# EnyaHermite/SPH3D-GCN

Hardware: AMD Instinct MI355X
Metric: point-cloud blocks/sec (fwd+bwd) SPH3D_s3dis 8192-pt (higher is better)
Workload: dtype f32

## Files before the change

### include/sph3d.h

```cpp
#ifndef SPH3D_H
#define SPH3D_H

#include <stddef.h>

#ifdef __cplusplus
extern "C" {
#endif

typedef void* sph3d_stream_t;

enum {
    SPH3D_OK = 0,
    SPH3D_EINVAL = -1,
    SPH3D_EWORKSPACE = -2,
    SPH3D_ELAUNCH = -3,
    SPH3D_EUNSUPPORTED = -4
};

#define SPH3D_ABI_VERSION 2
int sph3d_abi_version(void);
const char* sph3d_last_error(void);
const char* sph3d_build_info(void);


#define SPH3D_MAX_GROWTH_PASSES 4096
long long sph3d_nngrid_launches(void);
int sph3d_build_sphere_neighbor(int B, int N, int M, int nn_sample, float radius,
                                const float* database, const float* query,
                                int* nn_index, int* nn_count, float* nn_dist,
                                sph3d_stream_t stream);
int sph3d_build_sphere_neighbor_fixed(int B, int N, int M, int nn_sample, float radius,
                                const float* database, const float* query,
                                int* nn_index, int* nn_count, float* nn_dist,
                                sph3d_stream_t stream);

size_t sph3d_build_sphere_neighbor_workspace(int B, int N, int M);
int sph3d_build_sphere_neighbor_ws(int B, int N, int M, int nn_sample, float radius,
                                   const float* database, const float* query,
                                   int* nn_index, int* nn_count, float* nn_dist,
                                   void* workspace, size_t workspace_bytes, sph3d_stream_t stream);
int sph3d_build_sphere_neighbor_fixed_ws(int B, int N, int M, int nn_sample, float radius,
                                   const float* database, const float* query,
                                   int* nn_index, int* nn_count, float* nn_dist,
                                   void* workspace, size_t workspace_bytes, sph3d_stream_t stream);
int sph3d_release_stream_scratch(sph3d_stream_t stream);
int sph3d_release_all_scratch(void);

int sph3d_build_cube_neighbor(int B, int N, int M, int grid_size, int nn_sample, float length,
                              const float* database, const float* query,
                              int* nn_index, int* nn_count,
                              sph3d_stream_t stream);

int sph3d_build_sphere_graph(int B, int N, int M, int nn_sample, float radius, int n, int p, int q,
                             const float* database, const float* query,
                             int* nn_index, int* nn_count, float* nn_dist, int* filt_index,
                             void* transpose_workspace, size_t transpose_workspace_bytes, sph3d_stream_t stream);
int sph3d_build_sphere_graph_ocml(int B, int N, int M, int nn_sample, float radius, int n, int p, int q,
                             const float* database, const float* query,
                             int* nn_index, int* nn_count, float* nn_dist, int* filt_index,
                             void* transpose_workspace, size_t transpose_workspace_bytes, sph3d_stream_t stream);

int sph3d_build_sphere_graph_ws(int B, int N, int M, int nn_sample, float radius, int n, int p, int q, int ocml,
                                const float* database, const float* query,
                                int* nn_index, int* nn_count, float* nn_dist, int* filt_index,
                                void* transpose_workspace, size_t transpose_workspace_bytes,
                                void* search_workspace, size_t search_workspace_bytes, sph3d_stream_t stream);

int sph3d_spherical_kernel(int B, int N, int M, int K, int n, int p, int q, float radius,
                           const float* database, const float* query,
                           const int* nn_index, const int* nn_count, const float* nn_dist,
                           int* filt_index,
                           sph3d_stream_t stream);
int sph3d_spherical_kernel_ocml(int B, int N, int M, int K, int n, int p, int q, float radius,
                                const float* database, const float* query,
                                const int* nn_index, const int* nn_count, const float* nn_dist,
                                int* filt_index,
                                sph3d_stream_t stream);

int sph3d_depthwise_conv3d(int B, int N, int M, int F, int C, int r, int K,
                           const int* nn_index, const int* nn_count, const int* bin_index,
                           const float* input, const float* filter, float* output,
                           sph3d_stream_t stream);

size_t sph3d_depthwise_conv3d_grad_workspace(int B, int N, int M, int F, int C, int r, int K);
int sph3d_depthwise_conv3d_grad(int B, int N, int M, int F, int C, int r, int K,
                                const int* nn_index, const int* nn_count, const int* bin_index,
                                const float* input, const float* filter, const float* grad_output,
                                float* grad_input, float* grad_filter,
                                void* workspace, size_t workspace_bytes,
                                sph3d_stream_t stream);

size_t sph3d_graph_transpose_workspace(int B, int N, int M, int K, int F);
int sph3d_graph_transpose(int B, int N, int M, int K, int F,
                          const int* nn_index, const int* nn_count,
                          const int* bin_index , const float* weight ,
                          int* offsets, int* ent_key, float* ent_scale,
                          int* active_bins ,
                          void* workspace, size_t workspace_bytes, sph3d_stream_t stream);
int sph3d_graph_transpose_count(int B, int N, int M, int K, int F, const int* nn_index, const int* nn_count,
                                const int* bin_index, int want_active, void* workspace, size_t workspace_bytes,
                                sph3d_stream_t stream);
int sph3d_graph_transpose_finish(int B, int N, int M, int K, int F,
                                 const int* nn_index, const int* nn_count, const int* bin_index,
                                 const float* weight, int* offsets, int* ent_key, float* ent_scale, int* active_bins,
                                 void* workspace, size_t workspace_bytes, sph3d_stream_t stream);
int sph3d_gather_rows_count(int B, int N, int S, int K, const int* pairs, const int* nn_index, const int* nn_count,
                            int* out_index, int* out_count, void* transpose_workspace, size_t transpose_workspace_bytes,
                            sph3d_stream_t stream);
int sph3d_graph_transpose_finish_ordered(int B, int N, int M, int K, int F,
                                         const int* nn_index, const int* nn_count, const int* bin_index,
                                         const float* weight, int* offsets, int* ent_key, float* ent_scale, int* active_bins,
                                         int* order, void* workspace, size_t workspace_bytes, sph3d_stream_t stream);
int sph3d_graph_balanced_order(int B, int N, int F, const int* offsets, int* order, sph3d_stream_t stream);
size_t sph3d_depthwise_conv3d_grad_t_workspace(int B, int N, int F, int C, int r);
int sph3d_depthwise_conv3d_grad_t(int B, int N, int M, int F, int C, int r,
                                  const int* offsets, const int* ent_key, const float* ent_scale,
                                  const int* source_order ,
                                  const int* active_bins ,
                                  const float* input, const float* filter, const float* grad_output,
                                  float* grad_input, float* grad_filter,
                                  void* workspace, size_t workspace_bytes, sph3d_stream_t stream);
int sph3d_scatter_grad_t(int B, int Nin, int Mout, int C,
                         const int* offsets, const int* ent_key, const float* ent_scale,
                         const float* grad_output, float* grad_input, sph3d_stream_t stream);
size_t sph3d_scatter_grad_workspace(int B, int N, int M, int K);

int sph3d_max_pool3d(int B, int N, int M, int C, int K,
                     const int* nn_index, const int* nn_count, const float* input,
                     float* output, int* max_index, sph3d_stream_t stream);
int sph3d_max_pool3d_grad(int B, int N, int M, int C,
                          const int* max_index, const float* grad_output,
                          float* grad_input, sph3d_stream_t stream);
int sph3d_max_pool3d_grad_t(int B, int N, int M, int C, const int* offsets, const int* ent_key, const int* nn_count,
                            const int* max_index, const float* grad_output,
                            const float* addend ,
                            float* grad_input, sph3d_stream_t stream);
int sph3d_avg_pool3d(int B, int N, int M, int C, int K,
                     const int* nn_index, const int* nn_count, const float* input,
                     float* output, sph3d_stream_t stream);
int sph3d_avg_pool3d_grad(int B, int N, int M, int C, int K,
                          const int* nn_index, const int* nn_count, const float* grad_output,
                          float* grad_input,
                          void* workspace , size_t workspace_bytes,
                          sph3d_stream_t stream);

int sph3d_mean_interpolate(int B, int N, int M, int C, int K,
                           const int* nn_index, const int* nn_count, const float* input,
                           float* output, sph3d_stream_t stream);
int sph3d_mean_interpolate_grad(int B, int N, int M, int C, int K,
                                const int* nn_index, const int* nn_count, const float* grad_output,
                                float* grad_input,
                                void* workspace , size_t workspace_bytes,
                                sph3d_stream_t stream);
int sph3d_weighted_interpolate(int B, int N, int M, int C, int K,
                               const int* nn_index, const int* nn_count,
                               const float* input, const float* weight,
                               float* output, sph3d_stream_t stream);
int sph3d_weighted_interpolate_grad(int B, int N, int M, int C, int K,
                                    const int* nn_index, const int* nn_count,
                                    const float* grad_output, const float* weight,
                                    float* grad_input,
                                    void* workspace , size_t workspace_bytes,
                                    sph3d_stream_t stream);

size_t sph3d_farthest_point_sample_workspace(int b, int n, int m);
int sph3d_farthest_point_sample(int b, int n, int m, const float* inp, int* out,
                                void* workspace, size_t workspace_bytes,
                                sph3d_stream_t stream);

int sph3d_gather_nd(int B, int N, long long S, int row, const int* pairs, const void* params, void* out,
                    sph3d_stream_t stream);

int sph3d_spatial_order(int B, int N, const float* xyz, int* order, sph3d_stream_t stream);

int sph3d_pointwise_gemm(int R, int Cin, int Cout,
                         const float* X, const float* W, const float* bias, int act,
                         int trans_w, float* Y, sph3d_stream_t stream);
int sph3d_pointwise_gemm_mode(int mode);
int sph3d_pointwise_gemm_exchange_failures(void);
int sph3d_pointwise_gemm_tn(int R, int Cin, int Cout,
                            const float* X, const float* dY, float* dW,
                            void* workspace, size_t workspace_bytes,
                            sph3d_stream_t stream);
size_t sph3d_pointwise_gemm_tn_workspace(int R, int Cin, int Cout);

size_t sph3d_elu_bn_workspace(int R, int C);
int sph3d_elu_bn_forward(int R, int C, const float* y, const float* gamma, const float* beta,
                         float* running_mean, float* running_var, float momentum, float eps, int training,
                         float* out, float* save_mean, float* save_rstd,
                         void* workspace, size_t workspace_bytes, sph3d_stream_t stream);
int sph3d_elu_bn_backward(int R, int C, const float* y, const float* dout, const float* gamma,
                          const float* save_mean, const float* save_rstd, int training,
                          float* dy, float* dgamma, float* dbeta,
                          void* workspace, size_t workspace_bytes, sph3d_stream_t stream);

int sph3d_pointwise_gemm_bnstats_blocks(int R, int Cin, int Cout);
int sph3d_pointwise_gemm_bnstats(int R, int Cin, int Cout, const float* X, const float* W, const float* bias ,
                                 float* Y, float* partial, sph3d_stream_t stream);
int sph3d_elu_bn_forward_partials(int R, int C, int nblk, const float* partial, const float* y, const float* gamma,
                                  const float* beta, float* running_mean, float* running_var, float momentum, float eps,
                                  float* out, float* save_mean, float* save_rstd, sph3d_stream_t stream);

int sph3d_separable_conv3d_fused_supported(int N, int F, int C, int r, int K, int Cout);
int sph3d_separable_conv3d_fused(int B, int N, int M, int F, int C, int r, int K, int Cout, int act,
                                 const int* nn_index, const int* nn_count, const int* bin_index, const float* input,
                                 const float* depthwise_filter, const float* pointwise_weights, const float* bias,
                                 const float* scale, const float* shift, float* output, sph3d_stream_t stream);

int sph3d_separable_conv3d_train_supported(int N, int F, int C, int r, int K, int Cout);
int sph3d_separable_conv3d_train_blocks(int Cout);
int sph3d_separable_conv3d_train(int B, int N, int M, int F, int C, int r, int K, int Cout,
                                 const int* nn_index, const int* nn_count, const int* bin_index, const float* input,
                                 const float* depthwise_filter, const float* pointwise_weights, const float* bias,
                                 float* depthwise_output, float* y, float* partial, sph3d_stream_t stream);
int sph3d_separable_conv3d_ring_failures(void);

int sph3d_pointwise_gemm_skinny_supported(int R, int K1, int K2, int N);
int sph3d_pointwise_gemm_skinny(int R, int K1, int K2, int N, const float* A1, const float* A2, const float* W, const float* bias,
                                float* Y, sph3d_stream_t stream);
size_t sph3d_pointwise_gemm_skinny_tn_workspace(int R, int K1, int K2, int N);
int sph3d_pointwise_gemm_skinny_tn(int R, int K1, int K2, int N, const float* A1, const float* A2, const float* dY, float* dW,
                                   void* workspace, size_t workspace_bytes, sph3d_stream_t stream);

int sph3d_depthwise_conv3d_cat_supported(int F, int Ca, int Cb, int r);
int sph3d_depthwise_conv3d_cat(int B, int N, int M, int F, int Ca, int Cb, int r, int K, const int* nn_index, const int* nn_count,
                               const int* bin_index, const float* input_a, const float* input_b, const float* filter, float* output,
                               sph3d_stream_t stream);
int sph3d_depthwise_conv3d_grad_t_cat(int B, int N, int M, int F, int Ca, int Cb, int r, const int* offsets, const int* ent_key,
                                      const float* ent_scale, const int* source_order, const int* active_bins, const float* input_a,
                                      const float* input_b, const float* filter, const float* grad_output, float* grad_a,
                                      float* grad_b, float* grad_filter, void* workspace, size_t workspace_bytes,
                                      sph3d_stream_t stream);

int sph3d_adam_step(long long n, float* param, const float* grad, float* exp_avg, float* exp_avg_sq, float lr, float beta1,
                    float beta2, float eps, int step, sph3d_stream_t stream);

int sph3d_feed_assemble(int B, int num_point, int num_blocks, long long total_rows, const float* rows, const long long* offsets,
                        const int* block_ids, unsigned long long seed, unsigned long long step, int augment, float* points,
                        int* label, int* inner, int* index, sph3d_stream_t stream);

size_t sph3d_vote_workspace(long long batch_rows);
int sph3d_vote_begin(int B, int C, int num_blocks, long long total_rows, const float* rows, const long long* offsets,
                     const int* block_ids, long long row_base, long long batch_rows, float* votes, int* count, int* covered,
                     int* inner_size, int* remaining, void* workspace, size_t workspace_bytes, sph3d_stream_t stream);
int sph3d_vote_accumulate(int B, int num_point, int C, int num_blocks, long long total_rows, const float* rows,
                          const long long* offsets, const int* block_ids, long long row_base, long long batch_rows, int pass,
                          const int* index, const float* logits, int min_votes, float* votes, int* count, int* covered,
                          const int* inner_size, int* remaining, void* workspace, size_t workspace_bytes, sph3d_stream_t stream);
int sph3d_vote_finalize(int B, int C, int num_blocks, long long total_rows, const float* rows, const long long* offsets,
                        const int* block_ids, long long row_base, long long batch_rows, const float* votes, int* pred,
                        long long* confusion, long long* nonfinite, sph3d_stream_t stream);

#define SPH3D_NN1_GRID 0
#define SPH3D_NN1_BRUTE 1
int sph3d_scene_merge(int B, int C, int num_blocks, long long total_rows, const float* rows, const long long* offsets,
                      const int* index, const int* block_ids, long long row_base, long long batch_rows, const float* votes,
                      long long V, float* merged, int* hits, long long* counters, sph3d_stream_t stream);
int sph3d_scene_finalize(int C, long long V, const float* merged, const int* hits, const int* voxel_label, int* pred_voxel,
                         long long* unseen_rows, long long* confusion, sph3d_stream_t stream);
size_t sph3d_nn1_workspace(long long V, long long F);
int sph3d_nn1(long long V, long long F, const float* ref_xyz, const float* query_xyz, int mode, int* idx, void* workspace,
              size_t workspace_bytes, sph3d_stream_t stream);
int sph3d_scene_lift(int C, long long V, long long F, const int* pred_voxel, const int* idx, const int* label_map,
                     const int* label_full, int* pred_full, long long* confusion, sph3d_stream_t stream);

#define SPH3D_PREP_REDUCE_ATOMIC 0
#define SPH3D_PREP_REDUCE_SORTED 1
size_t sph3d_prep_voxel_grid_workspace(long long F, long long max_cells);
int sph3d_prep_voxel_grid(long long F, int A, const float* xyz, const float* attr, float h, long long max_cells,
                          int* voxel_of_point, int* header, void* workspace, size_t workspace_bytes, sph3d_stream_t stream);
size_t sph3d_prep_voxel_reduce_workspace(long long F, long long V, int mode);
int sph3d_prep_voxel_reduce(long long F, int A, long long V, const float* xyz, const float* attr, const int* voxel_of_point,
                            int mode, long long* sums, int* count, void* workspace, size_t workspace_bytes, sph3d_stream_t stream);
int sph3d_prep_voxel_finalize(long long V, int A, const long long* sums, const int* count, float* voxel_xyz, float* voxel_attr,
                              int* box, sph3d_stream_t stream);
int sph3d_prep_box(long long V, const float* xyz, int* box, sph3d_stream_t stream);
int sph3d_prep_normalise(long long V, const float* voxel_xyz, const float* voxel_rgb, const int* box, float* out_xyz,
                         float* out_rgb, sph3d_stream_t stream);
int sph3d_prep_rect_count(long long V, int R, const float* xyz, const float* rects, int* counts, sph3d_stream_t stream);
size_t sph3d_prep_block_fill_workspace(long long V, int P);
int sph3d_prep_block_fill(long long V, int P, long long T, const float* xyz, const float* rgb, const int* label,
                          const float* rects, const long long* offsets, float* rows, int* index, int* mismatch, void* workspace,
                          size_t workspace_bytes, sph3d_stream_t stream);

int sph3d_masked_softmax_xent_parts(int N);
int sph3d_masked_softmax_xent(int B, int N, int C, const float* logits, const long long* label, const float* inner_label,
                              float* loss_part, float* dlogits, sph3d_stream_t stream);

#ifdef __cplusplus
}
#endif
#endif
```

### sph3d_gcn_amd/_lib.py

```python
import ctypes
import os

import torch

_HERE = os.path.dirname(os.path.abspath(__file__))
LIB_PATH = os.environ.get("SPH3D_LIB") or os.path.join(_HERE, "csrc", "libsph3d.so")

_c_int = ctypes.c_int
_c_float = ctypes.c_float
_c_size_t = ctypes.c_size_t
_vp = ctypes.c_void_p

_I, _F, _P, _S, _L = _c_int, _c_float, _vp, _c_size_t, ctypes.c_longlong
SIGNATURES = {
    "sph3d_abi_version": (_I, []),
    "sph3d_last_error": (ctypes.c_char_p, []),
    "sph3d_build_info": (ctypes.c_char_p, []),
    "sph3d_build_sphere_neighbor": (_I, [_I, _I, _I, _I, _F, _P, _P, _P, _P, _P, _P]),
    "sph3d_build_sphere_neighbor_fixed": (_I, [_I, _I, _I, _I, _F, _P, _P, _P, _P, _P, _P]),
    "sph3d_build_sphere_neighbor_workspace": (_S, [_I, _I, _I]),
    "sph3d_build_sphere_neighbor_ws": (_I, [_I, _I, _I, _I, _F, _P, _P, _P, _P, _P, _P, _S, _P]),
    "sph3d_build_sphere_neighbor_fixed_ws": (_I, [_I, _I, _I, _I, _F, _P, _P, _P, _P, _P, _P, _S, _P]),
    "sph3d_release_stream_scratch": (_I, [_P]),
    "sph3d_release_all_scratch": (_I, []),
    "sph3d_build_sphere_graph_ws": (_I, [_I, _I, _I, _I, _F, _I, _I, _I, _I] + [_P] * 6 + [_P, _S, _P, _S, _P]),
    "sph3d_build_cube_neighbor": (_I, [_I, _I, _I, _I, _I, _F, _P, _P, _P, _P, _P]),
    "sph3d_spherical_kernel": (_I, [_I, _I, _I, _I, _I, _I, _I, _F, _P, _P, _P, _P, _P, _P, _P]),
    "sph3d_spherical_kernel_ocml": (_I, [_I, _I, _I, _I, _I, _I, _I, _F, _P, _P, _P, _P, _P, _P, _P]),
    "sph3d_depthwise_conv3d": (_I, [_I] * 7 + [_P] * 7),
    "sph3d_depthwise_conv3d_grad_workspace": (_S, [_I] * 7),
    "sph3d_depthwise_conv3d_grad": (_I, [_I] * 7 + [_P] * 8 + [_P, _S, _P]),
    "sph3d_max_pool3d": (_I, [_I] * 5 + [_P] * 6),
    "sph3d_max_pool3d_grad": (_I, [_I] * 4 + [_P] * 4),
    "sph3d_max_pool3d_grad_t": (_I, [_I] * 4 + [_P] * 8),
    "sph3d_avg_pool3d": (_I, [_I] * 5 + [_P] * 5),
    "sph3d_avg_pool3d_grad": (_I, [_I] * 5 + [_P] * 4 + [_P, _S, _P]),
    "sph3d_graph_balanced_order": (_I, [_I, _I, _I, _P, _P, _P]),
    "sph3d_gather_nd": (_I, [_I, _I, ctypes.c_longlong, _I, _P, _P, _P, _P]),
    "sph3d_gather_rows_count": (_I, [_I] * 4 + [_P] * 5 + [_P, _S, _P]),
    "sph3d_graph_transpose_workspace": (_S, [_I] * 5),
    "sph3d_graph_transpose": (_I, [_I] * 5 + [_P] * 8 + [_P, _S, _P]),
    "sph3d_graph_transpose_count": (_I, [_I] * 5 + [_P] * 3 + [_I, _P, _S, _P]),
    "sph3d_graph_transpose_finish": (_I, [_I] * 5 + [_P] * 8 + [_P, _S, _P]),
    "sph3d_graph_transpose_finish_ordered": (_I, [_I] * 5 + [_P] * 9 + [_P, _S, _P]),
    "sph3d_build_sphere_graph": (_I, [_I, _I, _I, _I, _F, _I, _I, _I] + [_P] * 6 + [_P, _S, _P]),
    "sph3d_build_sphere_graph_ocml": (_I, [_I, _I, _I, _I, _F, _I, _I, _I] + [_P] * 6 + [_P, _S, _P]),
    "sph3d_depthwise_conv3d_grad_t_workspace": (_S, [_I] * 5),
    "sph3d_depthwise_conv3d_grad_t": (_I, [_I] * 6 + [_P] * 10 + [_P, _S, _P]),
    "sph3d_depthwise_conv3d_cat_supported": (_I, [_I] * 4),
    "sph3d_depthwise_conv3d_cat": (_I, [_I] * 8 + [_P] * 8),
    "sph3d_depthwise_conv3d_grad_t_cat": (_I, [_I] * 7 + [_P] * 12 + [_P, _S, _P]),
    "sph3d_spatial_order": (_I, [_I, _I, _P, _P, _P]),
    "sph3d_scatter_grad_t": (_I, [_I] * 4 + [_P] * 6),
    "sph3d_scatter_grad_workspace": (_S, [_I] * 4),
    "sph3d_mean_interpolate": (_I, [_I] * 5 + [_P] * 5),
    "sph3d_mean_interpolate_grad": (_I, [_I] * 5 + [_P] * 4 + [_P, _S, _P]),
    "sph3d_weighted_interpolate": (_I, [_I] * 5 + [_P] * 6),
    "sph3d_weighted_interpolate_grad": (_I, [_I] * 5 + [_P] * 5 + [_P, _S, _P]),
    "sph3d_farthest_point_sample_workspace": (_S, [_I] * 3),
    "sph3d_farthest_point_sample": (_I, [_I] * 3 + [_P, _P, _P, _S, _P]),
    "sph3d_pointwise_gemm": (_I, [_I] * 3 + [_P, _P, _P, _I, _I, _P, _P]),
    "sph3d_pointwise_gemm_mode": (_I, [_I]),
    "sph3d_pointwise_gemm_tn_workspace": (_S, [_I] * 3),
    "sph3d_pointwise_gemm_tn": (_I, [_I] * 3 + [_P, _P, _P, _P, _S, _P]),
    "sph3d_elu_bn_workspace": (_S, [_I] * 2),
    "sph3d_pointwise_gemm_bnstats_blocks": (_I, [_I] * 3),
    "sph3d_pointwise_gemm_bnstats": (_I, [_I] * 3 + [_P] * 6),
    "sph3d_nngrid_launches": (ctypes.c_longlong, []),
    "sph3d_masked_softmax_xent_parts": (_I, [_I]),
    "sph3d_masked_softmax_xent": (_I, [_I, _I, _I] + [_P] * 5 + [_P]),
    "sph3d_adam_step": (_I, [ctypes.c_longlong] + [_P] * 4 + [_F] * 4 + [_I, _P]),
    "sph3d_feed_assemble": (_I, [_I, _I, _I, ctypes.c_longlong, _P, _P, _P, ctypes.c_ulonglong, ctypes.c_ulonglong, _I] + [_P] * 5),
    "sph3d_vote_workspace": (_S, [ctypes.c_longlong]),
    "sph3d_vote_begin": (_I, [_I, _I, _I, ctypes.c_longlong, _P, _P, _P, ctypes.c_longlong, ctypes.c_longlong] + [_P] * 5 + [_P, _S, _P]),
    "sph3d_vote_accumulate": (_I, [_I, _I, _I, _I, ctypes.c_longlong, _P, _P, _P, ctypes.c_longlong, ctypes.c_longlong, _I, _P, _P, _I]
                              + [_P] * 5 + [_P, _S, _P]),
    "sph3d_vote_finalize": (_I, [_I, _I, _I, ctypes.c_longlong, _P, _P, _P, ctypes.c_longlong, ctypes.c_longlong] + [_P] * 4 + [_P]),
    "sph3d_scene_merge": (_I, [_I, _I, _I, _L, _P, _P, _P, _P, _L, _L, _P, _L, _P, _P, _P, _P]),
    "sph3d_scene_finalize": (_I, [_I, _L] + [_P] * 6 + [_P]),
    "sph3d_nn1_workspace": (_S, [_L, _L]),
    "sph3d_nn1": (_I, [_L, _L, _P, _P, _I, _P, _P, _S, _P]),
    "sph3d_scene_lift": (_I, [_I, _L, _L] + [_P] * 6 + [_P]),
    "sph3d_prep_voxel_grid_workspace": (_S, [_L, _L]),
    "sph3d_prep_voxel_grid": (_I, [_L, _I, _P, _P, _F, _L, _P, _P, _P, _S, _P]),
    "sph3d_prep_voxel_reduce_workspace": (_S, [_L, _L, _I]),
    "sph3d_prep_voxel_reduce": (_I, [_L, _I, _L, _P, _P, _P, _I, _P, _P, _P, _S, _P]),
    "sph3d_prep_voxel_finalize": (_I, [_L, _I] + [_P] * 5 + [_P]),
    "sph3d_prep_box": (_I, [_L, _P, _P, _P]),
    "sph3d_prep_normalise": (_I, [_L] + [_P] * 5 + [_P]),
    "sph3d_prep_rect_count": (_I, [_L, _I, _P, _P, _P, _P]),
    "sph3d_prep_block_fill_workspace": (_S, [_L, _I]),
    "sph3d_prep_block_fill": (_I, [_L, _I, _L] + [_P] * 8 + [_P, _S, _P]),
    "sph3d_pointwise_gemm_skinny_supported": (_I, [_I] * 4),
    "sph3d_pointwise_gemm_skinny": (_I, [_I] * 4 + [_P] * 6),
    "sph3d_pointwise_gemm_skinny_tn_workspace": (_S, [_I] * 4),
    "sph3d_pointwise_gemm_skinny_tn": (_I, [_I] * 4 + [_P] * 5 + [_S, _P]),
    "sph3d_separable_conv3d_fused_supported": (_I, [_I] * 6),
    "sph3d_separable_conv3d_fused": (_I, [_I] * 9 + [_P] * 11),
    "sph3d_separable_conv3d_train_supported": (_I, [_I] * 6),
    "sph3d_separable_conv3d_train_blocks": (_I, [_I]),
    "sph3d_separable_conv3d_train": (_I, [_I] * 8 + [_P] * 11),
    "sph3d_separable_conv3d_ring_failures": (_I, []),
    "sph3d_pointwise_gemm_exchange_failures": (_I, []),
    "sph3d_elu_bn_forward_partials": (_I, [_I] * 3 + [_P] * 6 + [_F, _F] + [_P] * 4),
    "sph3d_elu_bn_forward": (_I, [_I, _I, _P, _P, _P, _P, _P, _F, _F, _I, _P, _P, _P, _P, _S, _P]),
    "sph3d_elu_bn_backward": (_I, [_I, _I] + [_P] * 5 + [_I] + [_P] * 3 + [_P, _S, _P]),
}
_EXTRA = {
    "sph3d_selftest_math": (_I, [_I, _P, _P, _P, _P, _P, _P, _P]),
}

ABI_VERSION = 2
_lib = None


class Sph3dError(RuntimeError):
    pass


def lib():
    global _lib
    if _lib is not None:
        return _lib
    if not os.path.exists(LIB_PATH):
        raise Sph3dError(
            "libsph3d.so is not built (%s).  Run `python -c 'import __graft_entry__ as g; g.build()'` "
            "or `make -C sph3d_gcn_amd/csrc`.  There is no fallback path." % LIB_PATH)
    l = ctypes.CDLL(LIB_PATH)
    for table in (SIGNATURES, _EXTRA):
        for name, (res, args) in table.items():
            try:
                fn = getattr(l, name)
            except AttributeError:
                if table is SIGNATURES:
                    raise Sph3dError("libsph3d.so does not export %s" % name)
                continue
            fn.restype = res
            fn.argtypes = args
    if l.sph3d_abi_version() != ABI_VERSION:
        raise Sph3dError("libsph3d.so ABI version %d, this package binds version %d" % (l.sph3d_abi_version(), ABI_VERSION))
    _lib = _Proxy(l)
    return _lib


_timing = None


def timing_start():
    global _timing
    _timing = []


def timing_stop():
    global _timing
    out, _timing = _timing, None
    return out


_PURE = ("_workspace", "_blocks", "_supported", "_parts")
_NO_TIME = ("sph3d_abi_version", "sph3d_last_error", "sph3d_build_info", "workspace", "_release_", "_blocks", "_supported", "_launches", "_parts", "_failures", "_mode")


class _Proxy:

    def __init__(self, cdll):
        self._cdll = cdll
        self._cache = {}

    def __getattr__(self, name):
        fn = getattr(self._cdll, name)
        if any(k in name for k in _PURE) and name != "sph3d_pointwise_gemm_bnstats_blocks":
            memo = {}

            def cached(*args, _fn=fn, _memo=memo):
                r = _memo.get(args)
                if r is None:
                    r = _memo[args] = _fn(*args)
                return r
            self.__dict__[name] = cached
            return cached
        if any(k in name for k in _NO_TIME):
            self.__dict__[name] = fn
            return fn
        w = self._cache.get(name)
        if w is None:
            sig = SIGNATURES.get(name) or _EXTRA.get(name)
            int_pos = tuple(i for i, t in enumerate(sig[1]) if t is _I) if sig else ()

            def w(*args, _fn=fn, _name=name, _pos=int_pos):
                if _timing is None:
                    return _fn(*args)
                st = torch.cuda.current_stream()
                e0 = torch.cuda.Event(enable_timing=True)
                e1 = torch.cuda.Event(enable_timing=True)
                e0.record(st)
                e0.raw_stream = st.cuda_stream
                rc = _fn(*args)
                e1.record(st)
                _timing.append((_name, tuple(args[i] for i in _pos if i < len(args)), e0, e1))
                return rc
            self._cache[name] = w
        self.__dict__[name] = w
        return w


def check(rc):
    if rc == 0:
        return
    msg = lib().sph3d_last_error().decode("utf-8", "replace")
    if rc == -1:
        raise ValueError(msg)
    raise Sph3dError("libsph3d status %d: %s" % (rc, msg))


_raw_stream = getattr(torch._C, "_cuda_getCurrentRawStream", None)
_get_device = getattr(torch._C, "_cuda_getDevice", None)


def current_raw_stream():
    if _raw_stream is not None and _get_device is not None:
        return _raw_stream(_get_device())
    return torch.cuda.current_stream().cuda_stream


def stream_ptr():
    return current_raw_stream()


def require_device(*tensors):
    for t in tensors:
        if not t.is_cuda:
            raise Sph3dError("sph3d ops run on the HIP device only (got a %s tensor); "
                             "the CPU oracle is test infrastructure, not a fallback" % t.device)


def f32(t):
    if t.dtype != torch.float32:
        t = t.float()
    return t.contiguous()


def i32(t):
    if t.dtype != torch.int32:
        t = t.int()
    return t.contiguous()


def ptr(t):
    return t.data_ptr() if t is not None else None


_scratch = {}


def release_scratch(stream=None):
    for key in [k for k in _scratch if stream is None or k[1] == stream]:
        del _scratch[key]


def scratch(nbytes, device, slot=0):
    if not nbytes:
        return None
    key = (device.index, current_raw_stream(), slot)
    t = _scratch.get(key)
    if t is None or t.numel() < nbytes:
        t = torch.empty((nbytes + nbytes // 4,), dtype=torch.uint8, device=device)
        _scratch[key] = t
    return t


class Arena:
    __slots__ = ("device", "cap", "off", "need", "_i32", "_f32", "buf")

    def __init__(self, nbytes, device):
        self.device, self.cap, self.off, self.need = device, int(nbytes), 0, 0
        self.buf = torch.empty((self.cap,), dtype=torch.uint8, device=device) if self.cap > 0 else None
        self._i32 = self.buf.view(torch.int32) if self.buf is not None else None
        self._f32 = self.buf.view(torch.float32) if self.buf is not None else None

    def take(self, shape, dtype):
        n = 4
        for d in shape:
            n *= d
        n = (n + 255) & ~255
        self.need += n
        if n == 0 or self.buf is None or self.off + n > self.cap:
            return None
        base = self._i32 if dtype is torch.int32 else self._f32
        strides, s = [], 1
        for d in reversed(shape):
            strides.append(s)
            s *= d
        strides.reverse()
        t = torch.as_strided(base, shape, strides, self.off >> 2)
        self.off += n
        return t


import threading

_arena = threading.local()


class arena_scope:

    def __init__(self, arena):
        self.arena = arena

    def __enter__(self):
        self.prev = getattr(_arena, "cur", None)
        _arena.cur = self.arena
        return self.arena

    def __exit__(self, *exc):
        _arena.cur = self.prev
        return False


def empty(shape, dtype, device):
    a = getattr(_arena, "cur", None)
    if a is not None and a.device == device and (dtype is torch.int32 or dtype is torch.float32):
        t = a.take(shape, dtype)
        if t is not None:
            return t
    return torch.empty(shape, dtype=dtype, device=device)
```

### sph3d_gcn_amd/csrc/nngrid.hip

```cpp
#include <atomic>
#include <cstdlib>
#include "common.hpp"
#include "sphere_bin.hpp"
#include "nnquery.hpp"

namespace sph3d {

typedef float f32x2 __attribute__((ext_vector_type(2)));

constexpr int kGridMaxCells = 8192;
constexpr int kGridMinCells = 512;
constexpr int kGridMaxK = 256;
constexpr int kGridMaxPos = 8;
constexpr int kGridReach = 3;

struct GridHdr {
    float minx, miny, minz, invh;
    int nx, ny, nz, nq;
};
constexpr int kMaxPositions = 64;
struct GridRadii {
    float thr[kMaxPositions], rk[kMaxPositions];
};

__device__ __forceinline__ int cell_of(float v, float lo, float invh, int n)
{
    const float t = floorf((v - lo) * invh);
    return t >= 0.0f ? (t < (float)n ? (int)t : n - 1) : 0;
}

__device__ __forceinline__ int block_excl_scan_1024(int v, int* tmp, int& total)
{
    const int lane = lane_id(), w = (int)threadIdx.x >> 6;
    const int ex = wave_excl_scan(v);
    __syncthreads();
    if (lane == 63) tmp[w] = ex + v;
    __syncthreads();
    int base = 0, tot = 0;
    for (int k = 0; k < 16; k++) {
        const int t = tmp[k];
        if (k < w) base += t;
        tot += t;
    }
    total = tot;
    return base + ex;
}

template <class CellOf, class Emit>
__device__ __forceinline__ void sort_by_cell(int n, int ncell, int* hist, int* tmp, int* cellStartOut, CellOf cellOf, Emit emit)
{
    const int tid = (int)threadIdx.x;
    for (int c = tid; c < ncell; c += 1024) hist[c] = 0;
    __syncthreads();
    for (int i = tid; i < n; i += 1024) atomicAdd(&hist[cellOf(i)], 1);
    __syncthreads();
    const int per = (ncell + 1023) / 1024;
    const int c0 = tid * per;
    int local = 0;
    for (int k = 0; k < per; k++)
        if (c0 + k < ncell) local += hist[c0 + k];
    int total;
    int run = block_excl_scan_1024(local, tmp, total);
    for (int k = 0; k < per; k++) {
        if (c0 + k < ncell) {
            const int c = hist[c0 + k];
            hist[c0 + k] = run;
            if (cellStartOut != nullptr) cellStartOut[c0 + k] = run;
            run += c;
        }
    }
    if (cellStartOut != nullptr && tid == 0) cellStartOut[ncell] = n;
    __syncthreads();
    for (int i = tid; i < n; i += 1024) emit(i, atomicAdd(&hist[cellOf(i)], 1));
    __syncthreads();
}

__global__ __launch_bounds__(1024) void nngrid_build_kernel(
    int N, int M, int npos, int fixed, float radius, const float* __restrict__ database,
    int* __restrict__ flag, GridRadii* __restrict__ radii, GridHdr* __restrict__ hdr, int* __restrict__ cellStart,
    float4* __restrict__ pts)
{
    extern __shared__ int hist[];
    __shared__ float redf[6][16];
    __shared__ int tmp[16];
    __shared__ GridHdr H;
    __shared__ int bad;
    const int b = (int)blockIdx.x, tid = (int)threadIdx.x, lane = lane_id(), w = tid >> 6;
    const float* db = database + (size_t)b * N * 3;
    if (tid == 0) bad = 0;
    float lo[3] = {INFINITY, INFINITY, INFINITY}, hi[3] = {-INFINITY, -INFINITY, -INFINITY};
    bool nonfinite = false;
    for (int i = tid; i < N; i += 1024) {
#pragma unroll
        for (int a = 0; a < 3; a++) {
            const float v = db[(size_t)i * 3 + a];
            nonfinite = nonfinite || !(fabsf(v) < INFINITY);
            lo[a] = fminf(lo[a], v);
            hi[a] = fmaxf(hi[a], v);
        }
    }
#pragma unroll
    for (int a = 0; a < 3; a++) {
        for (int o = 32; o > 0; o >>= 1) {
            lo[a] = fminf(lo[a], __shfl_xor(lo[a], o));
            hi[a] = fmaxf(hi[a], __shfl_xor(hi[a], o));
        }
        if (lane == 0) { redf[a][w] = lo[a]; redf[3 + a][w] = hi[a]; }
    }
    __syncthreads();
    if (nonfinite) bad = 1;
    __syncthreads();
    if (b == 0) {
        const int have = fixed ? 1 : (((int)gridDim.x + kRefGrid - 1) / kRefGrid) * ((M + kRefBlock - 1) / kRefBlock);
        for (int k0 = w; k0 < have; k0 += 16) {
            float rk = radius;
            for (int k = 0; k < k0; k++) rk = (float)((double)rk + 0.05);
            const float T = range_threshold(rk);
            if (lane == 0) { radii->thr[k0] = T; radii->rk[k0] = rk; }
        }
    }
    if (tid == 0) {
        float l3[3], h3[3];
        for (int a = 0; a < 3; a++) {
            l3[a] = redf[a][0]; h3[a] = redf[3 + a][0];
            for (int k = 1; k < 16; k++) { l3[a] = fminf(l3[a], redf[a][k]); h3[a] = fmaxf(h3[a], redf[3 + a][k]); }
        }
        const int maxCells = kGridMaxCells;
        float h = radius * 1.001f;
        int n3[3] = {0, 0, 0};
        bool ok = !bad && h > 0.0f && h < INFINITY;
        for (int it = 0; ok && it < 64; it++) {
            long long cells = 1;
            for (int a = 0; a < 3; a++) {
                const float e = (h3[a] - l3[a]) / h;
                if (!(e < 1.0e6f)) { cells = 1LL << 60; break; }
                n3[a] = (int)e + 1;
                cells *= n3[a];
            }
            if (cells <= maxCells) break;
            h *= cells > 8LL * maxCells ? 2.0f : 1.26f;
            if (it == 63) ok = false;
        }
        if (ok && (long long)n3[0] * n3[1] * n3[2] < kGridMinCells) ok = false;
        H.minx = l3[0]; H.miny = l3[1]; H.minz = l3[2];
        H.invh = 1.0f / h;
        H.nx = ok ? n3[0] : 0; H.ny = n3[1]; H.nz = n3[2];
        {
            const int S = (M + kRefBlock - 1) / kRefBlock;
            int sl = npos - (b / kRefGrid) * S;
            sl = sl < 0 ? 0 : (sl > S ? S : sl);
            H.nq = fixed ? M : (M < sl * kRefBlock ? M : sl * kRefBlock);
        }
        hdr[b] = H;
        if (!ok) *flag = 1;
    }
    __syncthreads();
    if (H.nx == 0) return;
    const int nx = H.nx, ny = H.ny, nz = H.nz, ncell = nx * ny * nz;
    const float mx = H.minx, my = H.miny, mz = H.minz, invh = H.invh;
    auto cell3 = [&](const float* p) {
        return (cell_of(p[0], mx, invh, nx) * ny + cell_of(p[1], my, invh, ny)) * nz + cell_of(p[2], mz, invh, nz);
    };
    float4* P = pts + (size_t)b * N;
    sort_by_cell(N, ncell, hist, tmp, cellStart + (size_t)b * (kGridMaxCells + 1),
                 [&](int i) { return cell3(db + (size_t)i * 3); },
                 [&](int i, int pos) {
                     P[pos] = make_float4(db[(size_t)i * 3], db[(size_t)i * 3 + 1], db[(size_t)i * 3 + 2], __int_as_float(i));
                 });
}

__global__ __launch_bounds__(1024) void nngrid_qorder_kernel(int M, int nslices, const float* __restrict__ query,
                                                             const GridHdr* __restrict__ hdr, int* __restrict__ qorder)
{
    extern __shared__ int hist[];
    __shared__ int tmp[16];
    const int b = (int)blockIdx.x / nslices, k = (int)blockIdx.x % nslices;
    const GridHdr H = hdr[b];
    const int j0 = k * kRefBlock;
    if (H.nx == 0 || j0 >= H.nq) return;
    const int n = H.nq - j0 < kRefBlock ? H.nq - j0 : kRefBlock;
    const int nx = H.nx, ny = H.ny, nz = H.nz;
    const float mx = H.minx, my = H.miny, mz = H.minz, invh = H.invh;
    const float* q = query + ((size_t)b * M + j0) * 3;
    int* qo = qorder + (size_t)b * M + j0;
    sort_by_cell(n, nx * ny * nz, hist, tmp, nullptr,
                 [&](int j) {
                     const float* p = q + (size_t)j * 3;
                     return (cell_of(p[0], mx, invh, nx) * ny + cell_of(p[1], my, invh, ny)) * nz + cell_of(p[2], mz, invh, nz);
                 },
                 [&](int j, int pos) { qo[pos] = j0 + j; });
}

__device__ __forceinline__ int quarter_excl_scan(int v)
{
    const int l16 = lane_id() & 15;
    int incl = v;
#pragma unroll
    for (int o = 1; o < 16; o <<= 1) {
        const int u = __shfl_up(incl, o, 16);
        if (l16 >= o) incl += u;
    }
    return incl - v;
}

template <bool FUSE>
__global__ __launch_bounds__(64) void nngrid_search_kernel(
    int B, int N, int M, int K, int W, int parts, int fixed, GraphFuse fx, int* __restrict__ flag,
    const GridRadii* __restrict__ radii, const GridHdr* __restrict__ hdr, const int* __restrict__ cellStart,
    const float4* __restrict__ pts, const int* __restrict__ qorder, const float* __restrict__ database,
    const float* __restrict__ query, int* __restrict__ nnIndex, int* __restrict__ nnCount, float* __restrict__ nnDist)
{
    extern __shared__ __attribute__((aligned(16))) unsigned char smem[];
    int b, part;
    xcd_decode((int)blockIdx.x, B, parts, b, part);
    if (b < 0) return;
    const GridHdr H = hdr[b];
    if (H.nx == 0 || part * 4 >= H.nq) return;
    const int lane = lane_id(), g = lane >> 4, l16 = lane & 15;
    unsigned* bm = reinterpret_cast<unsigned*>(smem) + (size_t)g * W;
    int2* bounds = reinterpret_cast<int2*>(smem + (size_t)4 * W * 4) + g * 64;
    unsigned short* list = reinterpret_cast<unsigned short*>(smem + (size_t)4 * W * 4 + 4 * 64 * 8) + (size_t)g * K;

    const int qpos = part * 4 + g;
    const bool valid = qpos < H.nq;
    const float4* P = pts + (size_t)b * N;
    const int* cs = cellStart + (size_t)b * (kGridMaxCells + 1);
    const float* db = database + (size_t)b * N * 3;
    int qid = 0, kq = 0;
    float qx = 0.f, qy = 0.f, qz = 0.f;
    if (valid) {
        qid = qorder[(size_t)b * M + qpos];
        const float* q = query + ((size_t)b * M + qid) * 3;
        qx = q[0]; qy = q[1]; qz = q[2];
        kq = fixed ? 0 : (b / kRefGrid) * ((M + kRefBlock - 1) / kRefBlock) + qid / kRefBlock;
    }
    const int nx = H.nx, ny = H.ny, nz = H.nz;
    const int cx = cell_of(qx, H.minx, H.invh, nx), cy = cell_of(qy, H.miny, H.invh, ny), cz = cell_of(qz, H.minz, H.invh, nz);
    const float T = radii->thr[kq];
    int c = (int)(radii->rk[kq] * H.invh) + 1;
    c = c > kGridReach ? kGridReach : c;
    const int side = 2 * c + 1;
    const int ncols = valid ? side * side : 0;
    const int zlo = cz - c > 0 ? cz - c : 0, zhi = cz + c < nz - 1 ? cz + c : nz - 1;

    for (int i = l16; i < W; i += 16) bm[i] = 0u;
    for (int ci = l16; ci < ncols; ci += 16) {
        const int X = cx + ci / side - c, Y = cy + ci % side - c;
        int2 be = make_int2(0, 0);
        if (X >= 0 && X < nx && Y >= 0 && Y < ny) {
            const int cb = (X * ny + Y) * nz;
            be.x = cs[cb + zlo];
            be.y = cs[cb + zhi + 1];
        }
        bounds[ci] = be;
    }
    __syncthreads();
    int col = 0, p = 0, e = 0;
    if (ncols > 0) { const int2 be = bounds[0]; p = be.x; e = be.y; }
    for (;;) {
        while (p >= e && col + 1 < ncols) {
            col++;
            const int2 be = bounds[col];
            p = be.x; e = be.y;
        }
        if (__builtin_amdgcn_ballot_w64(p < e) == 0ull) break;
        float4 cd[4];
        bool in[4];
#pragma unroll
        for (int u = 0; u < 4; u++) {
            const int i = p + u * 16 + l16;
            in[u] = i < e;
            cd[u] = P[in[u] ? i : 0];
        }
        p += 64;
#pragma unroll
        for (int u = 0; u < 4; u++) {
            const float dx = cd[u].x - qx, dy = cd[u].y - qy, dz = cd[u].z - qz;
            const float d2 = (dx * dx + dy * dy) + dz * dz;
            if (in[u] && d2 < T) {
                const unsigned id = (unsigned)__float_as_int(cd[u].w);
                atomicOr(&bm[id >> 5], 1u << (id & 31u));
            }
        }
    }
    __syncthreads();
    const int wpl = W / 16;
    int mine = 0;
    for (int i = 0; i < wpl; i++) mine += __popc(bm[l16 * wpl + i]);
    int rank = quarter_excl_scan(mine);
    const int found = __shfl(rank + mine, 15, 16);
    for (int i = 0; i < wpl && rank < K; i++) {
        unsigned word = bm[l16 * wpl + i];
        while (word != 0u && rank < K) {
            const int bit = __builtin_ctz(word);
            word &= word - 1u;
            list[rank++] = (unsigned short)((l16 * wpl + i) * 32 + bit);
        }
    }
    __syncthreads();
    const int cnt = found < K ? found : K;
    if (valid) {
        const size_t row = (size_t)b * M + qid;
        if (l16 == 0) {
            nnCount[row] = cnt;
            if (found == 0) *flag = 1;
        }
        for (int slot = l16; slot < K; slot += 16) {
            int id = 0, bin = 0;
            float dist = 0.0f;
            if (slot < cnt) {
                id = list[slot];
                const float dx = db[(size_t)id * 3] - qx;
                const float dy = db[(size_t)id * 3 + 1] - qy;
                const float dz = db[(size_t)id * 3 + 2] - qz;
                const float d2 = (dx * dx + dy * dy) + dz * dz;
                dist = sqrtf(sqrtf(d2));
                if (FUSE) {
                    if (fx.filt != nullptr)
                        bin = fx.ocml ? sphere_bin<true>(dx, dy, dz, dist, fx.radius, fx.n, fx.p, fx.q)
                                      : sphere_bin<false>(dx, dy, dz, dist, fx.radius, fx.n, fx.p, fx.q);
                    if (fx.deg != nullptr) {
                        fx.slotPos[row * K + slot] = atomicAdd(&fx.deg[((size_t)b * N + id) * fx.F + bin], 1);
                        fx.binUsed[bin] = 1;
                    }
                }
            }
            nnIndex[row * K + slot] = id;
            nnDist[row * K + slot] = dist;
            if (FUSE && fx.filt != nullptr) fx.filt[row * K + slot] = bin;
        }
    }
}

constexpr int kDenseQ = 4;
template <bool FUSE>
__global__ __launch_bounds__(256) void nndense_kernel(
    int B, int N, int M, int K, int j0, int parts, GraphFuse fx, int* __restrict__ flag, const GridRadii* __restrict__ radii,
    const GridHdr* __restrict__ hdr, const float* __restrict__ database, const float* __restrict__ query,
    int* __restrict__ nnIndex, int* __restrict__ nnCount, float* __restrict__ nnDist)
{
    extern __shared__ int lhits[];
    int b, part;
    xcd_decode((int)blockIdx.x, B, parts, b, part);
    if (b < 0 || hdr[b].nx == 0) return;
    const int lane = lane_id(), w = uniform((int)threadIdx.x >> 6);
    const int jw = j0 + (part * 4 + w) * kDenseQ;
    if (jw >= M) return;
    int* h = lhits + w * kDenseQ * K;
    const float* db = database + (size_t)b * N * 3;
    if (jw < hdr[b].nq) return;
    const float T = radii->thr[(b / kRefGrid) * ((M + kRefBlock - 1) / kRefBlock) + jw / kRefBlock];
    float qx[kDenseQ], qy[kDenseQ], qz[kDenseQ];
    int s[kDenseQ];
    bool live[kDenseQ];
#pragma unroll
    for (int c = 0; c < kDenseQ; c++) {
        live[c] = jw + c < M;
        const size_t row = (size_t)b * M + (live[c] ? jw + c : jw);
        qx[c] = query[row * 3]; qy[c] = query[row * 3 + 1]; qz[c] = query[row * 3 + 2];
        s[c] = live[c] ? 0 : K;
    }
    constexpr int S = 4;
    float px[S], py[S], pz[S];
    auto fetch = [&](int base, float* x, float* y, float* z) {
#pragma unroll
        for (int u = 0; u < S; u++) {
            const int i = base + u * 64 + lane;
            const int cl = i < N ? i : N - 1;
            x[u] = db[(size_t)cl * 3]; y[u] = db[(size_t)cl * 3 + 1]; z[u] = db[(size_t)cl * 3 + 2];
        }
    };
    fetch(0, px, py, pz);
    for (int base = 0; base < N; base += 64 * S) {
        bool open = false;
#pragma unroll
        for (int c = 0; c < kDenseQ; c++) open = open || s[c] < K;
        if (!open) break;
        float nx[S], ny[S], nz[S];
        const bool more = base + 64 * S < N;
        if (more) fetch(base + 64 * S, nx, ny, nz);
#pragma unroll
        for (int c = 0; c < kDenseQ; c++) {
            if (s[c] < K) {
                unsigned long long m[S];
                bool hit[S];
                unsigned long long any = 0ull;
#pragma unroll
                for (int u = 0; u < S; u += 2) {
                    const f32x2 dx = f32x2{px[u], px[u + 1]} - qx[c];
                    const f32x2 dy = f32x2{py[u], py[u + 1]} - qy[c];
                    const f32x2 dz = f32x2{pz[u], pz[u + 1]} - qz[c];
                    const f32x2 d2 = (dx * dx + dy * dy) + dz * dz;
                    hit[u] = base + u * 64 + lane < N && d2.x < T;
                    hit[u + 1] = base + (u + 1) * 64 + lane < N && d2.y < T;
                    m[u] = __builtin_amdgcn_ballot_w64(hit[u]);
                    m[u + 1] = __builtin_amdgcn_ballot_w64(hit[u + 1]);
                    any |= m[u] | m[u + 1];
                }
                if (any != 0ull) {
                    int sc = s[c];
#pragma unroll
                    for (int u = 0; u < S; u++) {
                        const int pos = sc + prefix_popc(m[u]);
                        if (hit[u] && pos < K) h[c * K + pos] = base + u * 64 + lane;
                        sc += __popcll(m[u]);
                    }
                    s[c] = sc;
                }
            }
        }
        if (more) {
#pragma unroll
            for (int u = 0; u < S; u++) { px[u] = nx[u]; py[u] = ny[u]; pz[u] = nz[u]; }
        }
    }
    __builtin_amdgcn_fence(__ATOMIC_RELEASE, "wavefront");
    __builtin_amdgcn_wave_barrier();
#pragma unroll 1
    for (int c = 0; c < kDenseQ; c++) {
        if (!live[c]) break;
        const size_t row = (size_t)b * M + jw + c;
        const int cnt = s[c] < K ? s[c] : K;
        if (lane == 0) {
            nnCount[row] = cnt;
            if (s[c] == 0) *flag = 1;
        }
        for (int slot = lane; slot < K; slot += 64) {
            int id = 0, bin = 0;
            float dist = 0.0f;
            if (slot < cnt) {
                id = h[c * K + slot];
                const float dx = db[(size_t)id * 3] - qx[c];
                const float dy = db[(size_t)id * 3 + 1] - qy[c];
                const float dz = db[(size_t)id * 3 + 2] - qz[c];
                const float d2 = (dx * dx + dy * dy) + dz * dz;
                dist = sqrtf(sqrtf(d2));
                if (FUSE) {
                    if (fx.filt != nullptr)
                        bin = fx.ocml ? sphere_bin<true>(dx, dy, dz, dist, fx.radius, fx.n, fx.p, fx.q)
                                      : sphere_bin<false>(dx, dy, dz, dist, fx.radius, fx.n, fx.p, fx.q);
                    if (fx.deg != nullptr) {
                        fx.slotPos[row * K + slot] = atomicAdd(&fx.deg[((size_t)b * N + id) * fx.F + bin], 1);
                        fx.binUsed[bin] = 1;
                    }
                }
            }
            nnIndex[row * K + slot] = id;
            nnDist[row * K + slot] = dist;
            if (FUSE && fx.filt != nullptr) fx.filt[row * K + slot] = bin;
        }
    }
}

static std::atomic<long long> g_grid_launches{0};

size_t nngrid_workspace_bytes(int B, int N, int M)
{
    if (B <= 0 || N <= 0 || M <= 0) return 0;
    if (N < 1024 || N > 65536 || M < 64 || M > kMaxPositions * kRefBlock || (long long)N * M < (1LL << 22)) return 0;
    const size_t hdrBytes = 1024 + sizeof(GridHdr) * (size_t)B;
    const size_t csBytes = sizeof(int) * (size_t)B * (kGridMaxCells + 1);
    const size_t ptBytes = sizeof(float4) * (size_t)B * N;
    const size_t qoBytes = sizeof(int) * (size_t)B * M;
    const size_t a16 = 15;
    return ((hdrBytes + a16) & ~a16) + ((csBytes + a16) & ~a16) + ptBytes + qoBytes;
}

int nngrid_search(int B, int N, int M, int K, float radius, int fixed, const float* database, const float* query, int* nn_index,
                  int* nn_count, float* nn_dist, const GraphFuse* fuse, hipStream_t st, const int** gate, int* grid_done,
                  void* workspace, size_t workspace_bytes, bool library_scratch)
{
    if (N < 1024 || N > 65536 || M < 64 || M > kMaxPositions * kRefBlock || (long long)N * M < (1LL << 22) || K > kGridMaxK ||
        (!fixed && B > kRefGrid && ((M >= kRefBlock && M % kRefBlock != 0) ||
                                    ((B + kRefGrid - 1) / kRefGrid) * ((M + kRefBlock - 1) / kRefBlock) > kMaxPositions)))
        return 0;
    int npos = 1;
    if (!fixed) {
        float rk = radius;
        while (npos < kGridMaxPos) {
            rk = (float)((double)rk + 0.05);
            if (!(rk <= kGridReach * radius)) break;
            npos++;
        }
        const int have = ((B + kRefGrid - 1) / kRefGrid) * ((M + kRefBlock - 1) / kRefBlock);
        if (npos > have) npos = have;
    }
    const size_t hdrBytes = 1024 + sizeof(GridHdr) * (size_t)B;
    const size_t csBytes = sizeof(int) * (size_t)B * (kGridMaxCells + 1);
    const size_t ptBytes = sizeof(float4) * (size_t)B * N;
    const size_t qoBytes = sizeof(int) * (size_t)B * M;
    const size_t a16 = 15;
    const size_t total = ((hdrBytes + a16) & ~a16) + ((csBytes + a16) & ~a16) + ptBytes + qoBytes;
    unsigned char* ws = (unsigned char*)workspace;
    if (ws != nullptr) {
        if (workspace_bytes < total || (reinterpret_cast<size_t>(ws) & 15) != 0) {
            set_error("BuildSphereNeighbor: workspace %zu B < required %zu B (or not 16-byte aligned)", workspace_bytes, total);
            return SPH3D_EWORKSPACE;
        }
    } else if (library_scratch) {
        ws = (unsigned char*)stream_scratch(st, total);
    }
    if (ws == nullptr) return 0;
    int* flag = (int*)ws;
    GridRadii* radii = (GridRadii*)(ws + 64);
    GridHdr* hdr = (GridHdr*)(ws + 1024);
    int* cellStart = (int*)(ws + ((hdrBytes + a16) & ~a16));
    float4* pts = (float4*)((unsigned char*)cellStart + ((csBytes + a16) & ~a16));
    int* qorder = (int*)((unsigned char*)pts + ptBytes);
    int rc = check_hip(hipMemsetAsync(flag, 0, 16, st), "nngrid: memset");
    if (rc) return rc;
    const size_t ldsBuild = sizeof(int) * (size_t)kGridMaxCells;
    hipLaunchKernelGGL(nngrid_build_kernel, dim3(B), dim3(1024), ldsBuild, st, N, M, npos, fixed, radius, database, flag,
                       radii, hdr, cellStart, pts);
    const int nq = fixed ? M : (M < npos * kRefBlock ? M : npos * kRefBlock);
    const int nslices = (nq + kRefBlock - 1) / kRefBlock;
    hipLaunchKernelGGL(nngrid_qorder_kernel, dim3(B * nslices), dim3(1024), ldsBuild, st, M, nslices, query, hdr, qorder);
    const int parts = (nq + 3) / 4;
    const int W = ((N + 31) / 32 + 15) & ~15;
    const size_t lds = (size_t)4 * W * 4 + 4 * 64 * 8 + (size_t)4 * K * 2;
    GraphFuse fx{};
    if (fuse != nullptr) fx = *fuse;
#define SPH3D_GRID(FU)                                                                                                      \
    do {                                                                                                                    \
        auto kern = nngrid_search_kernel<FU>;                                                                               \
        hipLaunchKernelGGL(kern, dim3(xcd_grid(B, parts)), dim3(64), lds, st, B, N, M, K, W, parts, fixed, fx, flag, radii, \
                           hdr, cellStart, pts, qorder, database, query, nn_index, nn_count, nn_dist);                      \
    } while (0)
    if (fuse != nullptr) SPH3D_GRID(true); else SPH3D_GRID(false);
#undef SPH3D_GRID
    int j0 = M;
    if (!fixed) {
        const int S = (M + kRefBlock - 1) / kRefBlock;
        int sl = npos - ((B - 1) / kRefGrid) * S;
        sl = sl < 0 ? 0 : (sl > S ? S : sl);
        j0 = sl * kRefBlock < M ? sl * kRefBlock : M;
    }
    if (j0 < M) {
        const int dparts = (M - j0 + 4 * kDenseQ - 1) / (4 * kDenseQ);
        const size_t dlds = sizeof(int) * 4 * kDenseQ * (size_t)K;
        if (fuse != nullptr)
            hipLaunchKernelGGL(nndense_kernel<true>, dim3(xcd_grid(B, dparts)), dim3(256), dlds, st, B, N, M, K, j0, dparts, fx, flag,
                               radii, hdr, database, query, nn_index, nn_count, nn_dist);
        else
            hipLaunchKernelGGL(nndense_kernel<false>, dim3(xcd_grid(B, dparts)), dim3(256), dlds, st, B, N, M, K, j0, dparts, fx, flag,
                               radii, hdr, database, query, nn_index, nn_count, nn_dist);
    }
    rc = check_launch("nngrid_search");
    if (rc) return rc;
    g_grid_launches.fetch_add(1, std::memory_order_relaxed);
    *gate = flag;
    *grid_done = 1 << 20;
    return 1;
}

}

extern "C" long long sph3d_nngrid_launches(void) { return sph3d::g_grid_launches.load(std::memory_order_relaxed); }
```

### sph3d_gcn_amd/csrc/nnquery.hip

```cpp
#include "common.hpp"
#include "sphere_bin.hpp"
#include "nnquery.hpp"

namespace sph3d {

typedef float f32x2 __attribute__((ext_vector_type(2)));

constexpr int kWavesPerWG = 16;
constexpr int kMaxChunk = 12288;
constexpr int kThrTable = 64;

constexpr float kPadCoord = 3.0e38f;
__device__ __forceinline__ int strip_off(int k, int comp) { return (k >> 7) * 384 + comp * 128 + (k & 127); }

__device__ __forceinline__ void stage_cloud(const float* __restrict__ dbi, int c0, int cn, float* lds)
{
    const float* src = dbi + (size_t)c0 * 3;
    for (int e = threadIdx.x; e < cn * 3; e += blockDim.x) {
        const float v = src[e];
        const int pnt = e / 3;
        const int comp = e - pnt * 3;
        lds[strip_off(pnt, comp)] = v;
    }
    const int cpad = (cn + 127) & ~127;
    for (int e = cn * 3 + (int)threadIdx.x; e < cpad * 3; e += blockDim.x) {
        const int pnt = e / 3;
        const int comp = e - pnt * 3;
        lds[strip_off(pnt, comp)] = kPadCoord;
    }
}

extern "C" __device__ int sph3d_writelane_i32(int val, int lane, int old) __asm("llvm.amdgcn.writelane.i32");
__device__ __forceinline__ int write_lane(int old, int val, int lane) { return sph3d_writelane_i32(val, lane, old); }


template <int CPW, bool MULTI, bool DEFER, bool FUSE>
__global__ __launch_bounds__(kWavesPerWG * 64) void nnquery_sphere_kernel(
    int B, int N, int M, int K, float radius0, int chunkN, int groups, int fixed, GraphFuse fx,
    const float* __restrict__ database, const float* __restrict__ query,
    int* __restrict__ nnIndex, int* __restrict__ nnCount, float* __restrict__ nnDist, const int* __restrict__ gate, int gridDone)
{
    const int kstart = (gate != nullptr && *gate == 0) ? gridDone : 0;
    if ((long long)kstart * kRefBlock >= M) return;
    extern __shared__ __attribute__((aligned(16))) float lds[];
    int* lhits = reinterpret_cast<int*>(lds + 3 * ((chunkN + 127) & ~127));
    float* lthr = reinterpret_cast<float*>(lhits + (DEFER ? kWavesPerWG * CPW * K : 0));
    {
        const int w = (int)threadIdx.x >> 6;
        float rk = radius0;
        for (int k = 0; k < kThrTable; k++) {
            if ((k & (kWavesPerWG - 1)) == w) {
                const float T = range_threshold(rk);
                if (lane_id() == 0) lthr[k] = T;
            }
            rk = (float)((double)rk + 0.05);
        }
        __syncthreads();
    }

    const int nt = M < kRefBlock ? M : kRefBlock;
    const int bb = (int)blockIdx.x / groups;
    const int g = (int)blockIdx.x % groups;
    const int wave = uniform((int)threadIdx.x >> 6);
    const int lane = lane_id();

    int t[CPW];
    float r[CPW];
    int kpos[CPW];
#pragma unroll
    for (int c = 0; c < CPW; c++) {
        t[c] = (g * kWavesPerWG + wave) * CPW + c;
        r[c] = radius0;
        kpos[c] = kstart;
    }
    for (int k = 0; k < kstart; k++) {
#pragma unroll
        for (int c = 0; c < CPW; c++) r[c] = (float)((double)r[c] + 0.05);
    }

    auto threshold_of = [&](int c) -> float {
        return kpos[c] < kThrTable ? uniformf(lthr[kpos[c]]) : range_threshold(r[c]);
    };

    for (int i = bb; i < B; i += kRefGrid) {
        const float* dbi = database + (size_t)i * N * 3;
        const float* qi = query + (size_t)i * M * 3;

        int j[CPW], s[CPW], passes[CPW];
        bool has[CPW];
        float qx[CPW], qy[CPW], qz[CPW], thr[CPW];
#pragma unroll
        for (int c = 0; c < CPW; c++) {
            j[c] = t[c] + kstart * kRefBlock;
            has[c] = (t[c] < nt) && (j[c] < M);
            s[c] = 0;
            passes[c] = 0;
            qx[c] = qy[c] = qz[c] = 0.0f;
            thr[c] = 0.0f;
            if (fixed) { r[c] = radius0; kpos[c] = 0; }
            if (has[c]) {
                qx[c] = qi[j[c] * 3];
                qy[c] = qi[j[c] * 3 + 1];
                qz[c] = qi[j[c] * 3 + 2];
                thr[c] = threshold_of(c);
            }
        }

        if (!MULTI) {
            __syncthreads();
            stage_cloud(dbi, 0, N, lds);
            __syncthreads();
        }

        int rec[CPW][4];
        int written[CPW];
#pragma unroll
        for (int c = 0; c < CPW; c++) {
            rec[c][0] = rec[c][1] = rec[c][2] = rec[c][3] = 0;
            written[c] = 0;
        }
        int wtrip = 0, wbase = 0;
        auto flush_hits = [&](int c) {
            if (s[c] == written[c]) return;
            unsigned long long m0 = (unsigned long long)(unsigned)rec[c][0] | ((unsigned long long)(unsigned)rec[c][1] << 32);
            unsigned long long m1 = (unsigned long long)(unsigned)rec[c][2] | ((unsigned long long)(unsigned)rec[c][3] << 32);
            int pos = written[c] + wave_excl_scan(__popcll(m0) + __popcll(m1));
            int* h = lhits + (wave * CPW + c) * K;
            const int id0 = wbase + lane * 128;
            while (m0 != 0ull && pos < K) {
                h[pos++] = id0 + (int)__builtin_ctzll(m0);
                m0 &= m0 - 1ull;
            }
            while (m1 != 0ull && pos < K) {
                h[pos++] = id0 + 64 + (int)__builtin_ctzll(m1);
                m1 &= m1 - 1ull;
            }
            written[c] = s[c];
            rec[c][0] = rec[c][1] = rec[c][2] = rec[c][3] = 0;
        };

        while (true) {
            bool any = false;
#pragma unroll
            for (int c = 0; c < CPW; c++) any = any || has[c];
            if (MULTI) any = __syncthreads_or(any ? 1 : 0) != 0;
            if (!any) break;

            wtrip = 0;
            wbase = 0;
            bool act[CPW];
#pragma unroll
            for (int c = 0; c < CPW; c++) act[c] = has[c] && s[c] < K;
            for (int c0 = 0; c0 < N; c0 += chunkN) {
                const int cn = (N - c0) < chunkN ? (N - c0) : chunkN;
                if (MULTI) {
                    __syncthreads();
                    stage_cloud(dbi, c0, cn, lds);
                    __syncthreads();
                }
                if constexpr (DEFER) {
                    unsigned long long am[CPW];
                    bool open = false;
#pragma unroll
                    for (int c = 0; c < CPW; c++) {
                        am[c] = act[c] ? ~0ull : 0ull;
                        open = open || act[c];
                    }
                    for (int base = 0; open && base < cn; base += 128) {
                        const float* sp = lds + (base >> 7) * 384 + lane;
                        const f32x2 x = {sp[0], sp[64]}, y = {sp[128], sp[192]}, z = {sp[256], sp[320]};
                        unsigned long long m0[CPW], m1[CPW], any = 0ull;
#pragma unroll
                        for (int c = 0; c < CPW; c++) {
                            const f32x2 dx = x - qx[c];
                            const f32x2 dy = y - qy[c];
                            const f32x2 dz = z - qz[c];
                            const f32x2 d2 = (dx * dx + dy * dy) + dz * dz;
                            m0[c] = __builtin_amdgcn_ballot_w64(d2.x < thr[c]) & am[c];
                            m1[c] = __builtin_amdgcn_ballot_w64(d2.y < thr[c]) & am[c];
                            any |= m0[c] | m1[c];
                        }
                        if (any != 0ull) {
#pragma unroll
                            for (int c = 0; c < CPW; c++) {
                                if ((m0[c] | m1[c]) != 0ull) {
                                    rec[c][0] = write_lane(rec[c][0], (int)(unsigned)m0[c], wtrip);
                                    rec[c][1] = write_lane(rec[c][1], (int)(unsigned)(m0[c] >> 32), wtrip);
                                    rec[c][2] = write_lane(rec[c][2], (int)(unsigned)m1[c], wtrip);
                                    rec[c][3] = write_lane(rec[c][3], (int)(unsigned)(m1[c] >> 32), wtrip);
                                    s[c] += __popcll(m0[c]) + __popcll(m1[c]);
                                    if (s[c] >= K) am[c] = 0ull;
                                }
                            }
                            unsigned long long o = 0ull;
#pragma unroll
                            for (int c = 0; c < CPW; c++) o |= am[c];
                            open = o != 0ull;
                        }
                        if (++wtrip == 64) {
#pragma unroll
                            for (int c = 0; c < CPW; c++) flush_hits(c);
                            wtrip = 0;
                            wbase = c0 + base + 128;
                        }
                    }
#pragma unroll
                    for (int c = 0; c < CPW; c++) {
                        flush_hits(c);
                        act[c] = has[c] && s[c] < K;
                    }
                    wtrip = 0;
                    wbase = c0 + cn;
                } else {
                    for (int base = 0; base < cn; base += 128) {
                        bool open = false;
#pragma unroll
                        for (int c = 0; c < CPW; c++) open = open || act[c];
                        if (!open) break;
                        const float* sp = lds + (base >> 7) * 384 + lane;
                        const f32x2 x = {sp[0], sp[64]}, y = {sp[128], sp[192]}, z = {sp[256], sp[320]};
#pragma unroll
                        for (int c = 0; c < CPW; c++) {
                            if (act[c]) {
                                const f32x2 dx = x - qx[c];
                                const f32x2 dy = y - qy[c];
                                const f32x2 dz = z - qz[c];
                                const f32x2 d2 = (dx * dx + dy * dy) + dz * dz;
                                const unsigned long long m0 = __builtin_amdgcn_ballot_w64(d2.x < thr[c]);
                                const unsigned long long m1 = __builtin_amdgcn_ballot_w64(d2.y < thr[c]);
                                if ((m0 | m1) != 0ull) {
                                    const bool hit0 = (m0 >> lane) & 1ull, hit1 = (m1 >> lane) & 1ull;
                                    const int pos0 = s[c] + prefix_popc(m0);
                                    const int pos1 = s[c] + __popcll(m0) + prefix_popc(m1);
                                    const size_t o = ((size_t)i * M + j[c]) * K;
                                    if (hit0 && pos0 < K) {
                                        nnIndex[o + pos0] = c0 + base + lane;
                                        nnDist[o + pos0] = sqrtf(sqrtf(d2.x));
                                    }
                                    if (hit1 && pos1 < K) {
                                        nnIndex[o + pos1] = c0 + base + 64 + lane;
                                        nnDist[o + pos1] = sqrtf(sqrtf(d2.y));
                                    }
                                    s[c] += __popcll(m0) + __popcll(m1);
                                    act[c] = s[c] < K;
                                }
                            }
                        }
                    }
                }
            }

#pragma unroll
            for (int c = 0; c < CPW; c++) {
                if (has[c]) {
                    r[c] = (float)((double)r[c] + 0.05);
                    kpos[c]++;
                    passes[c]++;
                    if (s[c] > 0 || passes[c] >= SPH3D_MAX_GROWTH_PASSES) {
                        const int cnt = s[c] < K ? s[c] : K;
                        const size_t row = (size_t)i * M + j[c];
                        if (lane == 0) nnCount[row] = cnt;
                        if (DEFER) {
                            const int* h = lhits + (wave * CPW + c) * K;
                            for (int slot = lane; slot < K; slot += 64) {
                                int id = 0, bin = 0;
                                float dist = 0.0f;
                                if (slot < cnt) {
                                    id = h[slot];
                                    const float dx = dbi[(size_t)id * 3] - qx[c];
                                    const float dy = dbi[(size_t)id * 3 + 1] - qy[c];
                                    const float dz = dbi[(size_t)id * 3 + 2] - qz[c];
                                    const float d2 = (dx * dx + dy * dy) + dz * dz;
                                    dist = sqrtf(sqrtf(d2));
                                    if (FUSE) {
                                        if (fx.filt != nullptr)
                                            bin = fx.ocml ? sphere_bin<true>(dx, dy, dz, dist, fx.radius, fx.n, fx.p, fx.q)
                                                          : sphere_bin<false>(dx, dy, dz, dist, fx.radius, fx.n, fx.p, fx.q);
                                        if (fx.deg != nullptr) {
                                            fx.slotPos[row * K + slot] = atomicAdd(&fx.deg[((size_t)i * N + id) * fx.F + bin], 1);
                                            fx.binUsed[bin] = 1;
                                        }
                                    }
                                }
                                nnIndex[row * K + slot] = id;
                                nnDist[row * K + slot] = dist;
                                if (FUSE && fx.filt != nullptr) fx.filt[row * K + slot] = bin;
                            }
                        } else {
                            for (int slot = cnt + lane; slot < K; slot += 64) {
                                nnIndex[row * K + slot] = 0;
                                nnDist[row * K + slot] = 0.0f;
                            }
                        }
                        j[c] += kRefBlock;
                        has[c] = j[c] < M;
                        s[c] = 0;
                        written[c] = 0;
                        passes[c] = 0;
                        if (fixed) { r[c] = radius0; kpos[c] = 0; }
                        if (has[c]) {
                            qx[c] = qi[j[c] * 3];
                            qy[c] = qi[j[c] * 3 + 1];
                            qz[c] = qi[j[c] * 3 + 2];
                        }
                    }
                    if (has[c]) thr[c] = threshold_of(c);
                }
            }
        }
    }
}

__global__ __launch_bounds__(256) void nnquery_cube_kernel(
    int B, int N, int M, int G, int K, float length,
    const float* __restrict__ database, const float* __restrict__ query,
    int* __restrict__ nnIndex, int* __restrict__ nnCount)
{
    const int lane = lane_id();
    const int wid = uniform((int)((blockIdx.x * blockDim.x + threadIdx.x) >> 6));
    const int nwaves = (int)((gridDim.x * blockDim.x) >> 6);
    const float half = length / 2;
    const float cell = length / (float)G;
    for (long long qid = wid; qid < (long long)B * M; qid += nwaves) {
        const int i = (int)(qid / M);
        const float* dbi = database + (size_t)i * N * 3;
        const float qx = query[qid * 3], qy = query[qid * 3 + 1], qz = query[qid * 3 + 2];
        int* row = nnIndex + (size_t)qid * K * 2;
        int s = 0;
        for (int base = 0; base < N && s < K; base += 64) {
            const int k = base + lane;
            const bool inb = k < N;
            const int kk = inb ? k : N - 1;
            const float dx = dbi[kk * 3] - qx;
            const float dy = dbi[kk * 3 + 1] - qy;
            const float dz = dbi[kk * 3 + 2] - qz;
            const bool hit = inb && fabsf(dx) < half && fabsf(dy) < half && fabsf(dz) < half;
            const unsigned long long mask = __ballot(hit);
            if (mask != 0ull) {
                const int pos = s + prefix_popc(mask);
                if (hit && pos < K) {
                    const int xId = (int)((dx + half) / cell);
                    const int yId = (int)((dy + half) / cell);
                    const int zId = (int)((dz + half) / cell);
                    row[pos * 2] = k;
                    row[pos * 2 + 1] = xId * G * G + yId * G + zId;
                }
                s += __popcll(mask);
            }
        }
        const int cnt = s < K ? s : K;
        if (lane == 0) nnCount[qid] = cnt;
        for (int slot = cnt * 2 + lane; slot < K * 2; slot += 64) row[slot] = 0;
    }
}

__global__ void gated_zero_kernel(const int* __restrict__ gate, int* __restrict__ p, long long n)
{
    if (*gate == 0) return;
    for (long long i = (long long)blockIdx.x * blockDim.x + threadIdx.x; i < n; i += (long long)gridDim.x * blockDim.x) p[i] = 0;
}

static size_t hits_bytes(int CPW, int K)
{
    const size_t b = sizeof(int) * (size_t)kWavesPerWG * CPW * K;
    return b <= 40 * 1024 ? b : 0;
}

template <int CPW, bool MULTI, bool DEFER>
static int launch_sphere(int B, int N, int M, int K, float radius, int chunkN,
                         const float* database, const float* query,
                         int* nn_index, int* nn_count, float* nn_dist, hipStream_t stream, int fixed,
                         const GraphFuse* fuse = nullptr, const int* gate = nullptr, int grid_done = 0)
{
    const int nb = B < kRefGrid ? B : kRefGrid;
    const int nt = M < kRefBlock ? M : kRefBlock;
    const int groups = (nt + kWavesPerWG * CPW - 1) / (kWavesPerWG * CPW);
    const size_t lds = (size_t)3 * ((chunkN + 127) & ~127) * sizeof(float) + (DEFER ? hits_bytes(CPW, K) : 0) + kThrTable * sizeof(float);
    if constexpr (DEFER) {
        if (fuse != nullptr) {
            int rc = launch_lds(nnquery_sphere_kernel<CPW, MULTI, DEFER, true>, dim3(nb * groups), dim3(kWavesPerWG * 64), lds, stream, "nnquery",
                                B, N, M, K, radius, chunkN, groups, fixed, *fuse, database, query, nn_index, nn_count, nn_dist, gate, grid_done);
            if (rc) return rc;
            return check_launch("sph3d_build_sphere_graph");
        }
    }
    int rc = launch_lds(nnquery_sphere_kernel<CPW, MULTI, DEFER, false>, dim3(nb * groups), dim3(kWavesPerWG * 64), lds, stream, "nnquery",
                        B, N, M, K, radius, chunkN, groups, fixed, GraphFuse{}, database, query, nn_index, nn_count, nn_dist, gate, grid_done);
    if (rc) return rc;
    return check_launch("sph3d_build_sphere_neighbor");
}

}

using namespace sph3d;

static int sphere_neighbor(int fixed, int B, int N, int M, int nn_sample, float radius,
                           const float* database, const float* query,
                           int* nn_index, int* nn_count, float* nn_dist,
                           sph3d_stream_t stream, const GraphFuse* fuse = nullptr, bool* fused = nullptr,
                           void* search_ws = nullptr, size_t search_ws_bytes = 0, bool library_scratch = true)
{
    if (fused) *fused = false;
    SPH3D_REQUIRE(radius > 0, "Range search requires radius>0, got %g", (double)radius);
    SPH3D_REQUIRE(nn_sample > 0, "BuildSphereNeighbor requires nn_sample>0, got %d", nn_sample);
    SPH3D_REQUIRE(B >= 0 && N > 0 && M >= 0, "BuildSphereNeighbor: bad dims B=%d N=%d M=%d", B, N, M);
    if (B == 0 || M == 0) return SPH3D_OK;
    hipStream_t st = as_stream(stream);
    const long long chains = (long long)(B < kRefGrid ? B : kRefGrid) * (M < kRefBlock ? M : kRefBlock);
    const int cpw = chains >= 256LL * kWavesPerWG * 4 ? 4 : (chains >= 256LL * kWavesPerWG * 2 ? 2 : 1);
    size_t hb = hits_bytes(cpw, nn_sample);
    int maxChunk = (int)((160 * 1024 - kThrTable * 4 - hb) / 12) & ~127;
    if (maxChunk > kMaxChunk) maxChunk = kMaxChunk;
    int chunkN = N < maxChunk ? N : maxChunk;
    const bool multi = N > chunkN;
    if (multi) {
        hb = hits_bytes(1, nn_sample);
        maxChunk = (int)((160 * 1024 - kThrTable * 4 - hb) / 12) & ~127;
        if (maxChunk > kMaxChunk) maxChunk = kMaxChunk;
        chunkN = maxChunk;
    }
    if (fused) *fused = (fuse != nullptr) && hb != 0;
    if (hb == 0) fuse = nullptr;
    const int* gate = nullptr;
    int grid_done = 0;
    const int g = nngrid_search(B, N, M, nn_sample, radius, fixed, database, query, nn_index, nn_count, nn_dist, fuse, st, &gate,
                                &grid_done, search_ws, search_ws_bytes, library_scratch);
    if (g < 0) return g;
    if (g > 0 && fuse != nullptr && fuse->deg != nullptr) {
        const long long cnt = (long long)B * N * fuse->F + fuse->F;
        hipLaunchKernelGGL(gated_zero_kernel, dim3(256), dim3(256), 0, st, gate, fuse->deg, cnt);
    }
#define SPH3D_NN(CP, MU)                                                                                          \
    return hb ? launch_sphere<CP, MU, true>(B, N, M, nn_sample, radius, chunkN, database, query, nn_index, nn_count, nn_dist, st, fixed, fuse, gate, grid_done) \
              : launch_sphere<CP, MU, false>(B, N, M, nn_sample, radius, chunkN, database, query, nn_index, nn_count, nn_dist, st, fixed, nullptr, gate, grid_done)
    if (multi) { SPH3D_NN(1, true); }
    if (cpw == 4) { SPH3D_NN(4, false); }
    if (cpw == 2) { SPH3D_NN(2, false); }
    SPH3D_NN(1, false);
#undef SPH3D_NN
}

extern "C" int sph3d_build_sphere_neighbor(int B, int N, int M, int nn_sample, float radius,
                                           const float* database, const float* query,
                                           int* nn_index, int* nn_count, float* nn_dist,
                                           sph3d_stream_t stream)
{
    return sphere_neighbor(0, B, N, M, nn_sample, radius, database, query, nn_index, nn_count, nn_dist, stream);
}

extern "C" int sph3d_build_sphere_neighbor_fixed(int B, int N, int M, int nn_sample, float radius,
                                                 const float* database, const float* query,
                                                 int* nn_index, int* nn_count, float* nn_dist,
                                                 sph3d_stream_t stream)
{
    return sphere_neighbor(1, B, N, M, nn_sample, radius, database, query, nn_index, nn_count, nn_dist, stream);
}

extern "C" size_t sph3d_build_sphere_neighbor_workspace(int B, int N, int M) { return nngrid_workspace_bytes(B, N, M); }

extern "C" int sph3d_build_sphere_neighbor_ws(int B, int N, int M, int nn_sample, float radius,
                                              const float* database, const float* query,
                                              int* nn_index, int* nn_count, float* nn_dist,
                                              void* workspace, size_t workspace_bytes, sph3d_stream_t stream)
{
    return sphere_neighbor(0, B, N, M, nn_sample, radius, database, query, nn_index, nn_count, nn_dist, stream, nullptr, nullptr,
                           workspace, workspace_bytes, false);
}

extern "C" int sph3d_build_sphere_neighbor_fixed_ws(int B, int N, int M, int nn_sample, float radius,
                                                    const float* database, const float* query,
                                                    int* nn_index, int* nn_count, float* nn_dist,
                                                    void* workspace, size_t workspace_bytes, sph3d_stream_t stream)
{
    return sphere_neighbor(1, B, N, M, nn_sample, radius, database, query, nn_index, nn_count, nn_dist, stream, nullptr, nullptr,
                           workspace, workspace_bytes, false);
}

extern "C" int sph3d_spherical_kernel(int B, int N, int M, int K, int n, int p, int q, float radius,
                                      const float* database, const float* query,
                                      const int* nn_index, const int* nn_count, const float* nn_dist,
                                      int* filt_index, sph3d_stream_t stream);
extern "C" int sph3d_graph_transpose_count(int B, int N, int M, int K, int F, const int* nn_index, const int* nn_count,
                                           const int* bin_index, int want_active, void* workspace, size_t workspace_bytes,
                                           sph3d_stream_t stream);

static int build_sphere_graph_impl(bool ocml, int B, int N, int M, int nn_sample, float radius, int n, int p, int q,
                                   const float* database, const float* query,
                                   int* nn_index, int* nn_count, float* nn_dist, int* filt_index,
                                   void* transpose_workspace, size_t transpose_workspace_bytes, sph3d_stream_t stream,
                                   void* search_ws = nullptr, size_t search_ws_bytes = 0, bool library_scratch = true)
{
    const bool binned = filt_index != nullptr;
    if (binned) {
        SPH3D_REQUIRE(n > 2 && n % 2 == 0, "Need n_>2 and n_%%2==0, got %d", n);
        SPH3D_REQUIRE(p > 0 && p % 2 == 0, "Need p_>0 and p_%%2==0, got %d", p);
        SPH3D_REQUIRE(q > 0, "Need q_>0, got %d", q);
    } else {
        SPH3D_REQUIRE(transpose_workspace != nullptr, "build_sphere_graph: without bins the call must count (workspace)");
    }
    const int F = binned ? n * p * q + 1 : 1;
    GraphFuse fx{};
    fx.n = n; fx.p = p; fx.q = q; fx.F = F;
    fx.radius = radius;
    fx.filt = filt_index;
    fx.ocml = ocml ? 1 : 0;
    if (transpose_workspace != nullptr) {
        const size_t need = sph3d_graph_transpose_workspace(B, N, M, nn_sample, F);
        if (transpose_workspace_bytes < need) {
            set_error("build_sphere_graph: transpose workspace %zu B < required %zu B", transpose_workspace_bytes, need);
            return SPH3D_EWORKSPACE;
        }
        const TgWs w = tg_ws(transpose_workspace, B, N, M, nn_sample, F);
        fx.deg = w.deg;
        fx.binUsed = w.bin_used;
        fx.slotPos = w.slot_pos;
        int rc = zero_async(w.deg, sizeof(int) * w.zero_words, as_stream(stream), "build_sphere_graph: memset");
        if (rc) return rc;
    }
    bool fused = false;
    int rc = sphere_neighbor(0, B, N, M, nn_sample, radius, database, query, nn_index, nn_count, nn_dist, stream, &fx, &fused,
                             search_ws, search_ws_bytes, library_scratch);
    if (rc || fused) return rc;
    if (binned)
        rc = ocml ? sph3d_spherical_kernel_ocml(B, N, M, nn_sample, n, p, q, radius, database, query, nn_index, nn_count, nn_dist, filt_index, stream)
                  : sph3d_spherical_kernel(B, N, M, nn_sample, n, p, q, radius, database, query, nn_index, nn_count, nn_dist, filt_index, stream);
    if (rc || transpose_workspace == nullptr) return rc;
    return sph3d_graph_transpose_count(B, N, M, nn_sample, F, nn_index, nn_count, filt_index, binned ? 1 : 0, transpose_workspace,
                                       transpose_workspace_bytes, stream);
}

extern "C" int sph3d_build_sphere_graph(int B, int N, int M, int nn_sample, float radius, int n, int p, int q,
                                        const float* database, const float* query,
                                        int* nn_index, int* nn_count, float* nn_dist, int* filt_index,
                                        void* transpose_workspace, size_t transpose_workspace_bytes, sph3d_stream_t stream)
{
    return build_sphere_graph_impl(false, B, N, M, nn_sample, radius, n, p, q, database, query, nn_index, nn_count, nn_dist, filt_index,
                                   transpose_workspace, transpose_workspace_bytes, stream);
}

extern "C" int sph3d_build_sphere_graph_ocml(int B, int N, int M, int nn_sample, float radius, int n, int p, int q,
                                             const float* database, const float* query,
                                             int* nn_index, int* nn_count, float* nn_dist, int* filt_index,
                                             void* transpose_workspace, size_t transpose_workspace_bytes, sph3d_stream_t stream)
{
    return build_sphere_graph_impl(true, B, N, M, nn_sample, radius, n, p, q, database, query, nn_index, nn_count, nn_dist, filt_index,
                                   transpose_workspace, transpose_workspace_bytes, stream);
}

extern "C" int sph3d_build_sphere_graph_ws(int B, int N, int M, int nn_sample, float radius, int n, int p, int q, int ocml,
                                           const float* database, const float* query,
                                           int* nn_index, int* nn_count, float* nn_dist, int* filt_index,
                                           void* transpose_workspace, size_t transpose_workspace_bytes,
                                           void* search_workspace, size_t search_workspace_bytes, sph3d_stream_t stream)
{
    return build_sphere_graph_impl(ocml != 0, B, N, M, nn_sample, radius, n, p, q, database, query, nn_index, nn_count, nn_dist,
                                   filt_index, transpose_workspace, transpose_workspace_bytes, stream, search_workspace,
                                   search_workspace_bytes, false);
}

extern "C" int sph3d_build_cube_neighbor(int B, int N, int M, int grid_size, int nn_sample, float length,
                                         const float* database, const float* query,
                                         int* nn_index, int* nn_count, sph3d_stream_t stream)
{
    SPH3D_REQUIRE(length > 0, "Cube search requires length>0, got %g", (double)length);
    SPH3D_REQUIRE(nn_sample > 0, "BuildCubeNeighbor requires nn_sample>0, got %d", nn_sample);
    SPH3D_REQUIRE(grid_size > 0, "BuildCubeNeighbor requires grid_size>0, got %d", grid_size);
    SPH3D_REQUIRE(B >= 0 && N > 0 && M >= 0, "BuildCubeNeighbor: bad dims B=%d N=%d M=%d", B, N, M);
    if (B == 0 || M == 0) return SPH3D_OK;
    const long long q = (long long)B * M;
    long long blocks = (q + 3) / 4;
    if (blocks > 4096) blocks = 4096;
    hipLaunchKernelGGL(nnquery_cube_kernel, dim3((unsigned)blocks), dim3(256), 0, as_stream(stream),
                       B, N, M, grid_size, nn_sample, length, database, query, nn_index, nn_count);
    return check_launch("sph3d_build_cube_neighbor");
}
```

### sph3d_gcn_amd/csrc/nnquery.hpp

```cpp
#pragma once
#include "common.hpp"

namespace sph3d {

__device__ __forceinline__ bool in_range(float s, float r)
{
    return s < r && (double)fabsf(s - r) > 1e-6;
}

__device__ inline float range_threshold(float r)
{
    if (!in_range(0.0f, r)) return 0.0f;
    const unsigned lane = (unsigned)lane_id();
    unsigned lo = 0u;
    unsigned hi = 0x7f800000u;
    while (hi - lo > 1u) {
        const unsigned span = hi - lo;
        const unsigned step = span / 65u + 1u;
        const unsigned long long c = (unsigned long long)lo + (unsigned long long)step * (lane + 1u);
        const bool p = (c < hi) && in_range(sqrtf(__uint_as_float((unsigned)c)), r);
        const int nt = __popcll(__ballot(p));
        const unsigned long long nhi = (unsigned long long)lo + (unsigned long long)step * (unsigned)(nt + 1);
        if (nhi < hi) hi = (unsigned)nhi;
        lo = lo + step * (unsigned)nt;
    }
    return __uint_as_float(hi);
}

__device__ __forceinline__ int wave_excl_scan(int v)
{
    int incl = v;
#pragma unroll
    for (int o = 1; o < 64; o <<= 1) {
        const int u = __shfl_up(incl, o);
        if (lane_id() >= o) incl += u;
    }
    return incl - v;
}

struct GraphFuse {
    int n, p, q, F;
    float radius;
    int* filt;
    int* deg;
    int* slotPos;
    int* binUsed;
    int ocml;
};

int nngrid_search(int B, int N, int M, int K, float radius, int fixed, const float* database, const float* query, int* nn_index,
                  int* nn_count, float* nn_dist, const GraphFuse* fuse, hipStream_t stream, const int** gate, int* grid_done,
                  void* workspace, size_t workspace_bytes, bool library_scratch);
size_t nngrid_workspace_bytes(int B, int N, int M);


}
```

### sph3d_gcn_amd/harness/s3dis_net.py

```python
import copy
import types

import torch
import torch.nn.functional as F

from .. import _lib
from .. import sph3gcn_util as s3g_util


def s3dis_config(num_input=8192):
    c = types.SimpleNamespace()
    c.num_input = num_input
    c.num_cls = 13
    c.mlp = 64
    c.num_sample = [2048, 768, 384, 128]
    c.radius = [0.1, 0.2, 0.4, 0.8]
    c.nn_uplimit = [64, 64, 64, 64]
    c.channels = [[128, 128], [256, 256], [256, 256], [512, 512]]
    c.multiplier = [[2, 2], [2, 2], [2, 2], [2, 2]]
    c.weight_decay = None
    c.kernel = [8, 2, 2]
    c.binSize = 8 * 2 * 2 + 1
    c.normalize = True
    c.pool_method = 'max'
    c.unpool_method = 'mean'
    c.sample = 'FPS'
    c.with_bn = True
    c.with_bias = False
    return c


def scannet_config(num_input=65536):
    c = s3dis_config(num_input)
    c.num_cls = 21
    c.num_sample = [num_input // 4, num_input * 3 // 32, num_input * 3 // 64, num_input // 64]
    return c


def small_config(num_input=1024):
    c = s3dis_config(num_input)
    c.num_sample = [256, 64]
    c.radius = [0.1, 0.2]
    c.nn_uplimit = [32, 32]
    c.channels = [[32, 32], [64, 64]]
    c.multiplier = [[2, 2], [2, 1]]
    c.mlp = 16
    return c


def normalize_xyz(points):
    min_xyz, max_xyz = torch.aminmax(points, dim=1, keepdim=True)
    center = (max_xyz + min_xyz) / 2
    xy = points[:, :, 0:2] - center[:, :, 0:2]
    z = points[:, :, 2:]
    return torch.cat((xy, z), dim=2)


def _net_input(points, config):
    xyz = points[:, :, 0:3]
    norm_xyz = normalize_xyz(xyz) if config.normalize else xyz
    return torch.cat((norm_xyz, points[:, :, 6:]), dim=2)


def _separable_conv3d_block(net, list_channels, bin_size, nn_index, nn_count, filt_idx, name,
                            depth_multiplier=None, weight_decay=None, reuse=None, with_bn=True,
                            with_bias=True, is_training=None):
    for l, num_out_channels in enumerate(list_channels):
        scope = name + '_' + str(l + 1)
        net = s3g_util.separable_conv3d(net, num_out_channels, bin_size, depth_multiplier[l], scope, nn_index,
                                        nn_count, filt_idx, weight_decay=weight_decay, with_bn=with_bn,
                                        with_bias=with_bias, reuse=reuse, is_training=is_training)
    return net


_side_stream = {}
SAMPLING_STREAMS = 1
_USE_ARENA = True
_ARENA_NEED = {}


class GraphPlan:

    def __init__(self, points, config, overlap=True, points_ready=None, decoder=True, global_kernel=None, global_radius=100.0,
                 global_query=None, prepare_input=True, need_backward=None, xyz_transform=None):
        self.config = config
        self.need_backward = torch.is_grad_enabled() if need_backward is None else bool(need_backward)
        self.decoder = bool(decoder)
        self.global_kernel, self.global_radius, self.global_query = global_kernel, float(global_radius), global_query
        self._glob, self._glob_ev = None, None
        xyz = points[:, :, 0:3]
        self.use_side = bool(overlap and xyz.is_cuda)
        self.xyz_layers, self.indices, self.events = [xyz], [], []
        self._enc, self._dec = {}, {}
        self._enc_ev, self._dec_ev, self._pool_ev = {}, {}, {}
        self._synced = set()
        self.net_input = None
        self._in_key = None
        if self.use_side:
            self.main = torch.cuda.current_stream()
            streams = _side_stream.get(xyz.device)
            if streams is None:
                streams = _side_stream[xyz.device] = ([torch.cuda.Stream(device=xyz.device) for _ in range(SAMPLING_STREAMS)],
                                                      torch.cuda.Stream(device=xyz.device), [0])
            s_fps = streams[0][streams[2][0] % len(streams[0])]
            streams[2][0] += 1
            s_graph = streams[1]
            if points_ready is not None:
                s_fps.wait_event(points_ready)
                s_graph.wait_event(points_ready)
            else:
                s_fps.wait_stream(self.main)
                s_graph.wait_stream(self.main)
            points.record_stream(s_fps)
            points.record_stream(s_graph)
            if torch.is_tensor(global_query):
                global_query.record_stream(s_graph)
            akey = (tuple(points.shape), id(config), bool(decoder), self.need_backward)
            need = _ARENA_NEED.get(akey, (0, 0))
            with torch.cuda.stream(s_fps), _lib.arena_scope(_lib.Arena(need[0], xyz.device) if _USE_ARENA else None) as a_fps:
                xyz = xyz.contiguous()
                if xyz_transform is not None:
                    xyz = xyz_transform(xyz).contiguous()
                if isinstance(self.global_query, str):
                    self.global_query = xyz.mean(dim=1, keepdim=True)
                    self.global_query.record_stream(s_graph)
                self.xyz_layers[0] = xyz
                ev_xyz = torch.cuda.Event()
                ev_xyz.record(s_fps)
                self._xyz_ev = ev_xyz
                if prepare_input:
                    self.net_input = _net_input(points, config)
                    self._in_key = (points.data_ptr(), points._version, tuple(points.shape))
                    self._in_ev = torch.cuda.Event()
                    self._in_ev.record(s_fps)
                self._sampling_chain(s_fps)
            s_graph.wait_event(ev_xyz)
            for t in self.xyz_layers + self.indices:
                if torch.is_tensor(t):
                    t.record_stream(s_graph)
            with torch.cuda.stream(s_graph), _lib.arena_scope(_lib.Arena(need[1], xyz.device) if _USE_ARENA else None) as a_graph:
                self._build_all(s_graph)
            if _USE_ARENA:
                unit = lambda n: ((n + (n >> 4) + (32 << 20) - 1) >> 25) << 25 if n > (8 << 20) else n + (n >> 4)
                want = (unit(a_fps.need), unit(a_graph.need))
                if want[0] > need[0] or want[1] > need[1]:
                    _ARENA_NEED[akey] = (max(want[0], need[0]), max(want[1], need[1]))
                    while len(_ARENA_NEED) > 16:
                        _ARENA_NEED.pop(next(iter(_ARENA_NEED)))
        else:
            if xyz_transform is not None:
                self.xyz_layers[0] = xyz_transform(xyz)
            if isinstance(self.global_query, str):
                self.global_query = self.xyz_layers[0].mean(dim=1, keepdim=True)
            self._sampling_chain(None)

    def xyz0(self):
        if self.use_side:
            self._sync(("xyz0",), self._xyz_ev, [self.xyz_layers[0]] + ([self.global_query] if torch.is_tensor(self.global_query) else []))
        return self.xyz_layers[0]

    def _sampling_chain(self, side):
        config = self.config
        for l in range(len(config.radius)):
            if config.num_sample[l] > 1:
                cur = self.xyz_layers[-1]
                if config.sample == 'FPS':
                    sample_index = s3g_util.farthest_point_sample(config.num_sample[l], cur)
                elif config.sample == 'random':
                    sample_index = s3g_util.random_sample(config.num_sample[l], cur)
                else:
                    raise ValueError('Unknown sampling method.')
                B = cur.shape[0]
                batch_indices = torch.arange(B, dtype=torch.int32, device=cur.device).view(-1, 1, 1)
                indices = torch.cat([batch_indices.expand(B, config.num_sample[l], 1),
                                     sample_index.unsqueeze(2).to(torch.int32)], dim=2)
                self.indices.append(indices)
                self.xyz_layers.append(s3g_util.gather_nd(cur, indices))
            else:
                self.indices.append(None)
            if side is not None:
                ev = torch.cuda.Event()
                ev.record(side)
                self.events.append(ev)

    def _make_enc(self, l):
        c = self.config
        xyz = self.xyz_layers[l]
        idx, cnt, dst, filt = s3g_util.build_intra_graph(xyz, c.radius[l], c.nn_uplimit[l], c.kernel, **self._bw_kw())
        return dict(intra_idx=idx, intra_cnt=cnt, filt_idx=filt)

    def _bw_kw(self):
        return {} if self.need_backward else {"with_transpose": False}

    def _make_pool(self, l, g):
        fused = getattr(s3g_util, "gather_pooling_graph", None)
        if fused is not None and g["intra_idx"].is_cuda:
            g["inter_idx"], g["inter_cnt"] = fused(g["intra_idx"], g["intra_cnt"], self.indices[l],
                                                   with_transpose=self.config.pool_method == 'max' and self.need_backward)
            return
        g["inter_idx"] = s3g_util.gather_nd(g["intra_idx"], self.indices[l])
        g["inter_cnt"] = s3g_util.gather_nd(g["intra_cnt"], self.indices[l])
        if self.config.pool_method == 'max' and g["inter_idx"].is_cuda and self.need_backward:
            from .. import _tgraph
            _tgraph.transpose(g["inter_idx"], g["inter_cnt"], self.xyz_layers[l].shape[1], unique_rows=True)

    def _make_dec(self, l):
        c = self.config
        L = len(c.radius)
        radius, uplimit = c.radius[L - 1 - l], c.nn_uplimit[L - 1 - l]
        xyz_c, xyz_unpool = self.xyz_layers[L - l], self.xyz_layers[L - 1 - l]
        intra_idx, intra_cnt, intra_dst, filt_idx = s3g_util.build_intra_graph(xyz_c, radius, uplimit, c.kernel, **self._bw_kw())
        from .. import tf_nnquery
        if (self.need_backward and xyz_c.is_cuda and c.unpool_method == 'mean' and s3g_util.neighbor_fn is s3g_util.build_sphere_neighbor
                and tf_nnquery.get_radius_mode() == "compat"):
            inter_idx, inter_cnt, inter_dst = tf_nnquery.build_sphere_neighbor_counted(xyz_c, xyz_unpool, radius, uplimit)
        else:
            inter_idx, inter_cnt, inter_dst = s3g_util.neighbor_fn(xyz_c, xyz_unpool, radius=radius, nnsample=uplimit)
        return dict(intra_idx=intra_idx, intra_cnt=intra_cnt, filt_idx=filt_idx, inter_idx=inter_idx,
                    inter_cnt=inter_cnt, inter_dst=inter_dst)

    def _pretranspose(self, g, n_src_conv, n_src_unpool=None):
        if not self.need_backward:
            return
        from .. import _tgraph
        _tgraph.transpose(g["intra_idx"], g["intra_cnt"], n_src_conv, bin_index=g["filt_idx"],
                          num_bins=self.config.binSize)
        if n_src_unpool is not None and self.config.unpool_method == 'mean':
            _tgraph.transpose(g["inter_idx"], g["inter_cnt"], n_src_unpool)

    def _build_all(self, stream):
        c = self.config
        L = len(c.radius)

        def mark(table, key):
            ev = torch.cuda.Event()
            ev.record(stream)
            table[key] = ev

        def make_dec(l):
            if not self.decoder:
                return
            g = self._make_dec(l)
            n_c = self.xyz_layers[L - l].shape[1]
            self._pretranspose(g, n_c, n_src_unpool=n_c)
            self._dec[l] = g
            mark(self._dec_ev, l)

        g = self._make_enc(0)
        self._pretranspose(g, self.xyz_layers[0].shape[1])
        self._enc[0] = g
        mark(self._enc_ev, 0)
        for s in range(L):
            stream.wait_event(self.events[s])
            if c.num_sample[s] > 1:
                self._make_pool(s, self._enc[s])
                mark(self._pool_ev, s)
            if s + 1 < L:
                g = self._make_enc(s + 1)
                self._pretranspose(g, self.xyz_layers[s + 1].shape[1])
                self._enc[s + 1] = g
                mark(self._enc_ev, s + 1)
            make_dec(L - 1 - s)
        if self.global_kernel is not None:
            self._glob = self._make_global()
            self._glob_ev = torch.cuda.Event()
            self._glob_ev.record(stream)

    def _make_global(self):
        xyz = self.xyz_layers[-1]
        query = self.global_query if self.global_query is not None else xyz.mean(dim=1, keepdim=True)
        nn_idx, nn_cnt, nn_dst = s3g_util.build_global_graph(xyz, query, self.global_radius)
        filt = s3g_util.spherical_kernel(xyz, query, nn_idx, nn_cnt, nn_dst, self.global_radius, kernel=self.global_kernel)
        return dict(nn_idx=nn_idx, nn_cnt=nn_cnt, filt_idx=filt, query=query)

    def glob(self):
        if self.use_side:
            self._sync(("glob",), self._glob_ev, list(self._glob.values()) + [self.xyz_layers[-1]])
        elif self._glob is None:
            self._glob = self._make_global()
        return self._glob

    def _sync(self, key, ev, tensors):
        if key in self._synced:
            return
        self.main.wait_event(ev)
        for t in tensors:
            if torch.is_tensor(t):
                t.record_stream(self.main)
        self._synced.add(key)

    def input(self, points):
        if (self.use_side and self.net_input is not None
                and self._in_key == (points.data_ptr(), points._version, tuple(points.shape))):
            self._sync(("input",), self._in_ev, [self.net_input])
            return self.net_input
        return _net_input(points, self.config)

    def enc(self, l):
        if self.use_side:
            self._sync(("enc", l), self._enc_ev[l], [self._enc[l]["intra_idx"], self._enc[l]["intra_cnt"],
                                                     self._enc[l]["filt_idx"], self.xyz_layers[l]])
        elif l not in self._enc:
            self._enc[l] = self._make_enc(l)
        return self._enc[l]

    def pool(self, l):
        g = self.enc(l)
        if self.use_side:
            self._sync(("pool", l), self._pool_ev[l], [g["inter_idx"], g["inter_cnt"]] + self.xyz_layers[l + 1:l + 2])
        elif "inter_idx" not in g:
            self._make_pool(l, g)
        return g

    def dec(self, l):
        if self.use_side:
            self._sync(("dec", l), self._dec_ev[l], list(self._dec[l].values()))
        elif l not in self._dec:
            self._dec[l] = self._make_dec(l)
        return self._dec[l]


def build_graphs(points, config, overlap=True):
    plan = GraphPlan(points, config, overlap=overlap)
    for l in range(len(config.radius)):
        plan.enc(l)
        if config.num_sample[l] > 1:
            plan.pool(l)
    for l in range(len(config.radius)):
        plan.dec(l)
    return plan


def get_model(points, is_training, config=None, graphs=None, points_ready=None):
    end_points = {}
    reuse = None
    plan = graphs if graphs is not None else GraphPlan(points, config, points_ready=points_ready)
    net = plan.input(points)
    net = s3g_util.pointwise_conv3d(net, config.mlp, 'mlp1', weight_decay=config.weight_decay,
                                    with_bn=config.with_bn, with_bias=config.with_bias, reuse=reuse,
                                    is_training=is_training)
    encoder = []
    for l in range(len(config.radius)):
        g = plan.enc(l)
        net = _separable_conv3d_block(net, config.channels[l], config.binSize, g["intra_idx"], g["intra_cnt"],
                                      g["filt_idx"], 'conv' + str(l + 1), config.multiplier[l], reuse=reuse,
                                      weight_decay=config.weight_decay, with_bn=config.with_bn,
                                      with_bias=config.with_bias, is_training=is_training)
        if config.num_sample[l] > 1:
            g = plan.pool(l)
            net, skip = s3g_util.pool3d_with_skip(net, g["inter_idx"], g["inter_cnt"], method=config.pool_method,
                                                  scope='pool' + str(l + 1))
            encoder.append(skip)
        else:
            encoder.append(net)
    channels = list(reversed(config.channels))
    multiplier = list(reversed(config.multiplier))
    encoder.reverse()
    for l in range(len(channels)):
        g = plan.dec(l)
        net = _separable_conv3d_block(net, channels[l], config.binSize, g["intra_idx"], g["intra_cnt"],
                                      g["filt_idx"], 'deconv' + str(l + 1), multiplier[l], reuse=reuse,
                                      weight_decay=config.weight_decay, with_bn=config.with_bn,
                                      with_bias=config.with_bias, is_training=is_training)
        net = s3g_util.unpool3d(net, g["inter_idx"], g["inter_cnt"], g["inter_dst"], method=config.unpool_method,
                                scope='unpool' + str(l + 1))
        if l + 1 < len(channels):
            net = (net, encoder[l])
    end_points = _EndPoints(end_points)
    end_points.feats_parts = (net, encoder[len(channels) - 1])
    net = s3g_util.pointwise_conv3d_concat(net, encoder[len(channels) - 1], config.num_cls, scope='logits', with_bn=False,
                                           with_bias=config.with_bias, activation_fn=None, is_training=is_training)
    return net, end_points


class _EndPoints(dict):
    feats_parts = None

    def __missing__(self, key):
        if key == 'feats' and self.feats_parts is not None:
            self['feats'] = torch.cat(self.feats_parts, dim=2)
            return self['feats']
        raise KeyError(key)


class _MaskedXentFn(torch.autograd.Function):

    @staticmethod
    def forward(ctx, pred, label, inner_label):
        from .. import _lib
        B, N, C = pred.shape
        pred = _lib.f32(pred)
        label = label.reshape(B, N).long().contiguous()
        inner = inner_label.reshape(B, N).float().contiguous()
        S = _lib.lib().sph3d_masked_softmax_xent_parts(N)
        loss_part = torch.empty((B, S), dtype=torch.float32, device=pred.device)
        dlogits = torch.empty_like(pred) if ctx.needs_input_grad[0] else None
        _lib.check(_lib.lib().sph3d_masked_softmax_xent(B, N, C, _lib.ptr(pred), _lib.ptr(label), _lib.ptr(inner),
                                                        _lib.ptr(loss_part), _lib.ptr(dlogits), _lib.stream_ptr()))
        if dlogits is not None:
            ctx.save_for_backward(dlogits)
        return loss_part

    @staticmethod
    def backward(ctx, g):
        (dlogits,) = ctx.saved_tensors
        return dlogits * g[:, 0].reshape(-1, 1, 1), None, None


def get_loss(pred, label, end_points, inner_label):
    B, N, C = pred.shape
    if pred.is_cuda:
        return _MaskedXentFn.apply(pred, label, inner_label).sum()
    loss = F.cross_entropy(pred.reshape(-1, C), label.reshape(-1), reduction='none').reshape(B, N)
    mask = (inner_label > 0).to(loss.dtype)
    cnt = mask.sum(dim=1)
    per_block = (loss * mask).sum(dim=1) / cnt.clamp(min=1.0)
    per_block = torch.where(cnt > 0, per_block, torch.zeros_like(per_block))
    return per_block.sum()


class SPH3DS3DIS(torch.nn.Module):

    def __init__(self, config=None, device=None, seed=7):
        super().__init__()
        self.config = copy.deepcopy(config) if config is not None else s3dis_config()
        self.store = s3g_util.VariableStore(device=device, seed=seed)

    def forward(self, points, is_training=True, graphs=None, points_ready=None):
        with s3g_util.variable_store(self.store):
            return get_model(points, is_training, self.config, graphs=graphs, points_ready=points_ready)

    def loss(self, pred, label, inner_label):
        return get_loss(pred, label, None, inner_label)
```

### sph3d_gcn_amd/sph3gcn_util.py

```python
import contextlib
import math

import torch
import torch.nn.functional as F

from . import tf_conv3d, tf_pool3d, tf_unpool3d
from .tf_nnquery import build_sphere_neighbor, build_cube_neighbor
from .tf_sample import farthest_point_sample, inverse_density_sample, random_sample
from .tf_buildkernel import spherical_kernel
from . import tf_gemm, tf_norm, _lib

neighbor_fn = build_sphere_neighbor

elu = F.elu


class VariableStore(torch.nn.Module):

    def __init__(self, device=None, seed=None):
        super().__init__()
        self.params = torch.nn.ParameterDict()
        self._device = device
        self._gen = None
        if seed is not None:
            self._gen = torch.Generator(device="cpu")
            self._gen.manual_seed(seed)
        self._decay = []
        self._reg = []

    def _key(self, name):
        return name.replace(".", "_")

    def has(self, name):
        return self._key(name) in self.params

    def get_variable(self, name, shape, init_fn, trainable=True):
        key = self._key(name)
        if key in self.params:
            return self.params[key]
        t = torch.empty(*shape, dtype=torch.float32)
        init_fn(t, self._gen)
        if self._device is not None:
            t = t.to(self._device)
        p = torch.nn.Parameter(t, requires_grad=trainable)
        self.params[key] = p
        return p

    def get_buffer(self, name, shape, value):
        key = self._key(name)
        if not hasattr(self, "_buf_" + key):
            t = torch.full(shape, float(value), dtype=torch.float32)
            if self._device is not None:
                t = t.to(self._device)
            self.register_buffer("_buf_" + key, t)
        return getattr(self, "_buf_" + key)

    def collect_losses(self):
        if not self._decay:
            return None
        return l2_sum([self.params[self._key(name)] for name, _c in self._decay], [c for _n, c in self._decay])

    def regularization_loss(self):
        if not self._reg:
            return None
        return l2_sum([self.params[self._key(name)] for name in self._reg], [1.0] * len(self._reg))


_coef_cache = {}


def l2_sum(params, coefs):
    key = (tuple(float(c) for c in coefs), params[0].device)
    c = _coef_cache.get(key)
    if c is None:
        c = _coef_cache[key] = torch.tensor(key[0], dtype=torch.float32, device=params[0].device)
    return _L2SumList.apply(c, key[0], *params)


class _L2SumList(torch.autograd.Function):
    @staticmethod
    def forward(ctx, coef_t, coef_list, *params):
        ctx.coef_list = list(coef_list)
        ctx.save_for_backward(*params)
        sq = torch.stack(torch._foreach_norm([p.detach() for p in params])).square()
        return 0.5 * (sq * coef_t).sum()

    @staticmethod
    def backward(ctx, g):
        grads = torch._foreach_mul(list(ctx.saved_tensors), ctx.coef_list)
        grads = torch._foreach_mul(grads, g)
        return (None, None) + tuple(grads)


_default_store = VariableStore()
_active = [_default_store]


def get_variable_store():
    return _active[-1]


@contextlib.contextmanager
def variable_store(store):
    _active.append(store)
    try:
        yield store
    finally:
        _active.pop()


def _xavier_uniform(t, gen):
    shape = t.shape
    receptive = 1
    for s in shape[:-2]:
        receptive *= s
    fan_in = shape[-2] * receptive if len(shape) > 1 else shape[0]
    fan_out = shape[-1] * receptive
    limit = math.sqrt(6.0 / (fan_in + fan_out))
    with torch.no_grad():
        t.uniform_(-limit, limit, generator=gen)


def _truncated_normal(stddev):
    def init(t, gen):
        with torch.no_grad():
            torch.nn.init.trunc_normal_(t, mean=0.0, std=stddev, a=-2 * stddev, b=2 * stddev, generator=gen)
    return init


def _constant(value):
    def init(t, gen):
        with torch.no_grad():
            t.fill_(value)
    return init


def _variable_with_weight_decay(name, shape, stddev, with_decay, use_xavier=True):
    store = get_variable_store()
    new = not store.has(name)
    var = store.get_variable(name, shape, _xavier_uniform if use_xavier else _truncated_normal(stddev))
    if new and with_decay is not None:
        store._decay.append((name, with_decay))
    return var


def build_global_graph(xyz, query, radius):
    nn_uplimit = xyz.shape[1]
    nn_idx, nn_cnt, nn_dst = neighbor_fn(xyz, query, radius=radius, nnsample=nn_uplimit)
    return nn_idx, nn_cnt, nn_dst


def build_graph(xyz, radius, nn_uplimit, num_sample, sample_method=None):
    intra_idx, intra_cnt, intra_dst = neighbor_fn(xyz, xyz, radius=radius, nnsample=nn_uplimit)

    if num_sample is not None:
        if sample_method == 'random':
            sample_index = random_sample(num_sample, xyz)
        elif sample_method == 'FPS':
            sample_index = farthest_point_sample(num_sample, xyz)
        elif sample_method == 'IDS':
            prob = torch.sum(intra_dst, dim=-1) / intra_cnt.float()
            sample_index = inverse_density_sample(num_sample, prob)
        else:
            raise ValueError('Unknown sampling method.')

        batch_size = xyz.shape[0]
        batch_indices = torch.arange(batch_size, dtype=torch.int32, device=xyz.device).view(-1, 1, 1)
        batch_indices = batch_indices.expand(batch_size, num_sample, 1)
        indices = torch.cat([batch_indices, sample_index.unsqueeze(2).to(torch.int32)], dim=2)
    else:
        indices = None

    return intra_idx, intra_cnt, intra_dst, indices


def build_graph_deconv(xyz, xyz_unpool, radius, nn_uplimit):
    intra_idx, intra_cnt, intra_dst = neighbor_fn(xyz, xyz, radius=radius, nnsample=nn_uplimit)
    inter_idx, inter_cnt, inter_dst = neighbor_fn(xyz, xyz_unpool, radius=radius, nnsample=nn_uplimit)
    return intra_idx, intra_cnt, intra_dst, inter_idx, inter_cnt, inter_dst


def build_intra_graph(xyz, radius, nn_uplimit, kernel, with_transpose=True):
    from . import tf_nnquery
    if xyz.is_cuda and neighbor_fn is build_sphere_neighbor and tf_nnquery.get_radius_mode() == "compat":
        return tf_nnquery.build_sphere_graph(xyz, radius, nn_uplimit, kernel, with_transpose=with_transpose)
    idx, cnt, dst = neighbor_fn(xyz, xyz, radius=radius, nnsample=nn_uplimit)
    return idx, cnt, dst, spherical_kernel(xyz, xyz, idx, cnt, dst, radius, kernel=kernel)


def gather_nd(params, indices):
    if (params.is_cuda and params.dim() >= 2 and params.element_size() == 4 and indices.dtype == torch.int32
            and indices.shape[-1] == 2 and not params.requires_grad):
        params = params.contiguous()
        indices = indices.contiguous()
        B, N = params.shape[0], params.shape[1]
        row = 1
        for d in params.shape[2:]:
            row *= d
        S = indices.numel() // 2
        out = _lib.empty(tuple(indices.shape[:-1]) + tuple(params.shape[2:]), params.dtype, params.device)
        if S and row:
            _lib.check(_lib.lib().sph3d_gather_nd(B, N, S, row, _lib.ptr(indices), _lib.ptr(params), _lib.ptr(out),
                                                 _lib.stream_ptr()))
        return out
    b = indices[..., 0].long()
    p = indices[..., 1].long()
    return params[b, p]


def gather_pooling_graph(nn_index, nn_count, indices, with_transpose=True):
    if not (nn_index.is_cuda and nn_index.dim() == 3 and nn_count.dim() == 2 and indices.dtype == torch.int32 and indices.shape[-1] == 2
            and indices.shape[0] == nn_index.shape[0]):
        return gather_nd(nn_index, indices), gather_nd(nn_count, indices)
    from . import _tgraph
    nn_index, nn_count, indices = nn_index.contiguous(), nn_count.contiguous(), indices.contiguous()
    B, N, K = nn_index.shape
    S = indices.shape[1]
    dev = nn_index.device
    out_idx = _lib.empty((B, S, K), torch.int32, dev)
    out_cnt = _lib.empty((B, S), torch.int32, dev)
    l = _lib.lib()
    ws, wsb = None, 0
    if with_transpose:
        wsb = l.sph3d_graph_transpose_workspace(B, N, S, K, 1)
        ws = torch.empty((max(wsb, 1),), dtype=torch.uint8, device=dev)
    _lib.check(l.sph3d_gather_rows_count(B, N, S, K, _lib.ptr(indices), _lib.ptr(nn_index), _lib.ptr(nn_count), _lib.ptr(out_idx),
                                         _lib.ptr(out_cnt), _lib.ptr(ws), wsb, _lib.stream_ptr()))
    if with_transpose:
        _tgraph.transpose(out_idx, out_cnt, N, counted_workspace=ws, unique_rows=True)
    return out_idx, out_cnt


def _finish(outputs, num_out_channels, scope, activation_fn, with_bn, with_bias, reuse, is_training, fused_bias=None):
    if with_bias and fused_bias is None:
        biases = get_variable_store().get_variable(scope + '/biases', [num_out_channels], _constant(0.0))
        outputs = outputs + biases
    if (with_bn and activation_fn is elu and FUSE_ELU_BN and outputs.is_cuda and tf_norm.supported(outputs.shape[-1])):
        return _elu_batch_normalization(outputs, is_training, name=scope + '/bn')
    if activation_fn is not None:
        outputs = activation_fn(outputs)
    if with_bn:
        outputs = batch_normalization(outputs, is_training, name=scope + '/bn', reuse=reuse)
    return outputs


def _fused_tail_applies(x2d, num_out_channels, activation_fn, with_bn, with_bias, is_training):
    training = True if is_training is None else bool(is_training)
    return (FUSE_GEMM_BN and FUSE_ELU_BN and with_bn and activation_fn is elu and training and x2d.is_cuda
            and tf_norm.supported(num_out_channels)
            and tf_norm.gemm_bn_blocks(x2d.shape[0], x2d.shape[1], num_out_channels) > 0)


def _gemm_tail(x2d, kernel, out_shape, num_out_channels, scope, activation_fn, with_bn, with_bias, reuse, is_training):
    if _fused_tail_applies(x2d, num_out_channels, activation_fn, with_bn, with_bias, is_training):
        store = get_variable_store()
        biases = store.get_variable(scope + '/biases', [num_out_channels], _constant(0.0)) if with_bias else None
        gamma, beta, moving_mean, moving_var = _bn_variables(store, scope + '/bn', num_out_channels)
        out = tf_norm.gemm_elu_batch_norm(x2d, kernel, gamma, beta, moving_mean, moving_var, bias=biases)
        return out.reshape(out_shape)
    if (FUSE_GEMM_BN and with_bias and not with_bn and x2d.is_cuda and (activation_fn is elu or activation_fn is None)):
        biases = get_variable_store().get_variable(scope + '/biases', [num_out_channels], _constant(0.0))
        out = tf_gemm.matmul_bias_act(x2d, kernel, biases, elu=activation_fn is elu)
        return out.reshape(out_shape)
    outputs = tf_gemm.matmul(x2d, kernel).reshape(out_shape)
    return _finish(outputs, num_out_channels, scope, activation_fn, with_bn, with_bias, reuse, is_training)


def separable_conv3d(inputs,
                     num_out_channels,
                     kernel_size,
                     depth_multiplier,
                     scope,
                     nn_index,
                     nn_count,
                     filt_index,
                     use_xavier=True,
                     stddev=1e-3,
                     weight_decay=None,
                     activation_fn=elu,
                     with_bn=False,
                     with_bias=False,
                     reuse=None,
                     is_training=None):
    pair = inputs if isinstance(inputs, (tuple, list)) else None
    infer_fused = (FUSE_SEPARABLE_INFERENCE and is_training is not None and not bool(is_training) and not torch.is_grad_enabled()
                   and (activation_fn is elu or activation_fn is None))
    if pair is not None and infer_fused and pair[0].is_cuda and getattr(tf_conv3d, "separable_fused_supported_dims", None) is not None \
            and tf_conv3d.separable_fused_supported_dims(pair[0].shape[1], kernel_size, pair[0].shape[-1] + pair[1].shape[-1],
                                                         depth_multiplier, nn_index.shape[2], num_out_channels) \
            and (FUSE_SEPARABLE_INFERENCE is True
                 or _fused_rows_pay(nn_index.shape[0] * nn_index.shape[1], pair[0].shape[-1] + pair[1].shape[-1], depth_multiplier,
                                    num_out_channels)):
        inputs, pair = torch.cat(tuple(pair), dim=2), None
    if pair is not None:
        supported = getattr(tf_conv3d, "concat_supported", None)
        if not (FUSE_CONV_CONCAT and pair[0].is_cuda and supported is not None and supported(pair[0], pair[1], torch.empty(
                (kernel_size, pair[0].shape[-1] + pair[1].shape[-1], depth_multiplier), device='meta'))):
            inputs, pair = torch.cat(tuple(pair), dim=2), None
    num_in_channels = inputs.shape[-1] if pair is None else pair[0].shape[-1] + pair[1].shape[-1]
    depthwise_kernel = _variable_with_weight_decay(scope + '/depthwise_weights',
                                                   shape=[kernel_size, num_in_channels, depth_multiplier],
                                                   use_xavier=use_xavier, stddev=stddev,
                                                   with_decay=weight_decay)
    if pair is not None:
        outputs = tf_conv3d.depthwise_conv3d_concat(pair[0], pair[1], depthwise_kernel, nn_index, nn_count, filt_index)
        batch_size = outputs.shape[0]
        num_in_channels = outputs.shape[-1]
        kernel = _variable_with_weight_decay(scope + '/weights', shape=[num_in_channels, num_out_channels],
                                             use_xavier=use_xavier, stddev=stddev, with_decay=weight_decay)
        return _gemm_tail(outputs.reshape(-1, num_in_channels), kernel, (batch_size, -1, num_out_channels), num_out_channels, scope,
                          activation_fn, with_bn, with_bias, reuse, is_training)
    if (infer_fused and tf_conv3d.separable_fused_supported(inputs, depthwise_kernel, nn_index, num_out_channels)
            and (FUSE_SEPARABLE_INFERENCE is True or _fused_layer_pays(inputs, depth_multiplier, nn_index, num_out_channels))):
        store = get_variable_store()
        kernel = _variable_with_weight_decay(scope + '/weights', shape=[num_in_channels * depth_multiplier, num_out_channels],
                                             use_xavier=use_xavier, stddev=stddev, with_decay=weight_decay)
        biases = store.get_variable(scope + '/biases', [num_out_channels], _constant(0.0)) if with_bias else None
        scale = shift = None
        if with_bn:
            gamma, beta, moving_mean, moving_var = _bn_variables(store, scope + '/bn', num_out_channels)
            scale = gamma * torch.rsqrt(moving_var + 1e-3)
            shift = beta - moving_mean * scale
        return tf_conv3d.separable_conv3d_fused(inputs, depthwise_kernel, kernel, nn_index, nn_count, filt_index, bias=biases,
                                                elu=activation_fn is elu, scale=scale, shift=shift)
    training = True if is_training is None else bool(is_training)
    if (FUSE_SEPARABLE_TRAINING and training and with_bn and activation_fn is elu and FUSE_ELU_BN and inputs.is_cuda
            and getattr(tf_conv3d, "separable_train_supported", None) is not None
            and tf_conv3d.separable_train_supported(inputs, depthwise_kernel, nn_index, num_out_channels)
            and (FUSE_SEPARABLE_TRAINING is True
                 or _fused_train_pays(nn_index.shape[0] * nn_index.shape[1], num_in_channels, depth_multiplier, num_out_channels))):
        store = get_variable_store()
        kernel = _variable_with_weight_decay(scope + '/weights', shape=[num_in_channels * depth_multiplier, num_out_channels],
                                             use_xavier=use_xavier, stddev=stddev, with_decay=weight_decay)
        biases = store.get_variable(scope + '/biases', [num_out_channels], _constant(0.0)) if with_bias else None
        gamma, beta, moving_mean, moving_var = _bn_variables(store, scope + '/bn', num_out_channels)
        return tf_conv3d.separable_conv3d_elu_bn_train(inputs, depthwise_kernel, kernel, gamma, beta, moving_mean, moving_var,
                                                       nn_index, nn_count, filt_index, bias=biases)
    outputs = tf_conv3d.depthwise_conv3d(inputs, depthwise_kernel, nn_index, nn_count, filt_index)

    batch_size = outputs.shape[0]
    num_in_channels = outputs.shape[-1]
    kernel = _variable_with_weight_decay(scope + '/weights', shape=[num_in_channels, num_out_channels],
                                         use_xavier=use_xavier, stddev=stddev, with_decay=weight_decay)
    return _gemm_tail(outputs.reshape(-1, num_in_channels), kernel, (batch_size, -1, num_out_channels), num_out_channels, scope,
                      activation_fn, with_bn, with_bias, reuse, is_training)


def pointwise_conv3d(inputs,
                     num_out_channels,
                     scope,
                     use_xavier=True,
                     stddev=1e-3,
                     weight_decay=None,
                     activation_fn=elu,
                     with_bn=False,
                     with_bias=False,
                     reuse=None,
                     is_training=None):
    batch_size = inputs.shape[0]
    num_in_channels = inputs.shape[-1]
    kernel = _variable_with_weight_decay(scope + '/weights', shape=[num_in_channels, num_out_channels],
                                         use_xavier=use_xavier, stddev=stddev, with_decay=weight_decay)
    return _gemm_tail(inputs.reshape(-1, num_in_channels), kernel, (batch_size, -1, num_out_channels), num_out_channels, scope,
                      activation_fn, with_bn, with_bias, reuse, is_training)


def pointwise_conv3d_concat(inputs_a, inputs_b, num_out_channels, scope, use_xavier=True, stddev=1e-3, weight_decay=None,
                            activation_fn=elu, with_bn=False, with_bias=False, reuse=None, is_training=None):
    ca, cb = inputs_a.shape[-1], inputs_b.shape[-1]
    if (FUSE_LOGITS_CONCAT and inputs_a.is_cuda and not with_bn and activation_fn is None
            and tf_gemm.skinny_supported(inputs_a.shape[0] * inputs_a.shape[1], ca, cb, num_out_channels)):
        kernel = _variable_with_weight_decay(scope + '/weights', shape=[ca + cb, num_out_channels],
                                             use_xavier=use_xavier, stddev=stddev, with_decay=weight_decay)
        biases = get_variable_store().get_variable(scope + '/biases', [num_out_channels], _constant(0.0)) if with_bias else None
        out = tf_gemm.linear_concat2(inputs_a.reshape(-1, ca), inputs_b.reshape(-1, cb), kernel, biases)
        return out.reshape(inputs_a.shape[0], -1, num_out_channels)
    return pointwise_conv3d(torch.cat((inputs_a, inputs_b), dim=2), num_out_channels, scope, use_xavier=use_xavier, stddev=stddev,
                            weight_decay=weight_decay, activation_fn=activation_fn, with_bn=with_bn, with_bias=with_bias,
                            reuse=reuse, is_training=is_training)


def fully_connected(inputs,
                    num_out_channels,
                    scope,
                    use_xavier=True,
                    stddev=1e-3,
                    weight_decay=None,
                    activation_fn=elu,
                    with_bn=False,
                    with_bias=False,
                    reuse=None,
                    is_training=None):
    num_in_channels = inputs.shape[-1]
    kernel = _variable_with_weight_decay(scope + '/weights', shape=[num_in_channels, num_out_channels],
                                         use_xavier=use_xavier, stddev=stddev, with_decay=weight_decay)
    return _gemm_tail(inputs, kernel, (inputs.shape[0], num_out_channels), num_out_channels, scope, activation_fn, with_bn,
                      with_bias, reuse, is_training)


def pool3d(inputs, nn_index, nn_count, scope, method):
    if method == 'max':
        outputs, max_index = tf_pool3d.max_pool3d(inputs, nn_index, nn_count)
    elif method == 'avg':
        outputs = tf_pool3d.avg_pool3d(inputs, nn_index, nn_count)
    else:
        raise ValueError("Unknow pooling method %s." % method)
    return outputs


def pool3d_with_skip(inputs, nn_index, nn_count, scope, method):
    fn = getattr(tf_pool3d, "max_pool3d_with_skip", None)
    if method == 'max' and FUSE_POOL_SKIP and inputs.is_cuda and fn is not None:
        outputs, _max_index, skip = fn(inputs, nn_index, nn_count)
        return outputs, skip
    return pool3d(inputs, nn_index, nn_count, scope, method), inputs


def unpool3d(inputs, nn_index, nn_count, nn_dist, scope, method):
    if method == 'mean':
        outputs = tf_unpool3d.mean_interpolate(inputs, nn_index, nn_count)
    elif method == 'weighted':
        sum_nn_dist = torch.sum(nn_dist, dim=-1, keepdim=True)
        epsilon = 1e-7
        weight = (nn_dist + epsilon) / (sum_nn_dist + epsilon)
        outputs = tf_unpool3d.weighted_interpolate(inputs, weight, nn_index, nn_count)
    else:
        raise ValueError("Unknow unpooling method %s." % method)
    return outputs


FUSE_GEMM_BN = True
FUSE_POOL_SKIP = True
FUSE_CONV_CONCAT = True
FUSE_LOGITS_CONCAT = True
FUSE_SEPARABLE_INFERENCE = "auto"


FUSE_SEPARABLE_TRAINING = False
_FUSED_TRAIN_MIN_ROWS = 16384


def _fused_train_pays(rows, C, r, Cout):
    return rows >= _FUSED_TRAIN_MIN_ROWS


def _fused_rows_pay(rows, C, r, Cout):
    small = C <= 128 and C * r <= 256 and Cout <= 128
    return small or rows >= 16384


def _fused_layer_pays(inputs, depth_multiplier, nn_index, num_out_channels):
    return _fused_rows_pay(nn_index.shape[0] * nn_index.shape[1], inputs.shape[-1], depth_multiplier, num_out_channels)
FUSE_ELU_BN = True


def _bn_variables(store, name, C):
    new = not store.has(name + '/gamma')
    gamma = store.get_variable(name + '/gamma', [C], _constant(1.0))
    beta = store.get_variable(name + '/beta', [C], _constant(0.0))
    if new:
        store._reg.extend([name + '/gamma', name + '/beta'])
    moving_mean = store.get_buffer(name + '/moving_mean', (C,), 0.0)
    moving_var = store.get_buffer(name + '/moving_variance', (C,), 1.0)
    return gamma, beta, moving_mean, moving_var


def _elu_batch_normalization(data, is_training, name):
    store = get_variable_store()
    gamma, beta, moving_mean, moving_var = _bn_variables(store, name, data.shape[-1])
    training = True if is_training is None else bool(is_training)
    return tf_norm.elu_batch_norm(data, gamma, beta, moving_mean, moving_var, training)


def batch_normalization(data, is_training, name, reuse=None):
    store = get_variable_store()
    C = data.shape[-1]
    gamma, beta, moving_mean, moving_var = _bn_variables(store, name, C)
    training = True if is_training is None else bool(is_training)
    flat = data.reshape(-1, C)
    if training:
        out = F.batch_norm(flat, None, None, gamma, beta, training=True, momentum=0.0, eps=1e-3)
        with torch.no_grad():
            var, mean = torch.var_mean(flat, dim=0, unbiased=False)
            moving_mean.mul_(0.99).add_(mean, alpha=1.0 - 0.99)
            moving_var.mul_(0.99).add_(var, alpha=1.0 - 0.99)
    else:
        out = F.batch_norm(flat, moving_mean, moving_var, gamma, beta, training=False, momentum=0.0, eps=1e-3)
    return out.reshape(data.shape)
```

### sph3d_gcn_amd/tf_nnquery.py

```python
from typing import Tuple

import torch

from . import _lib

_radius_mode = "compat"


def get_radius_mode():
    return _radius_mode


def set_radius_mode(mode):
    global _radius_mode
    if mode not in ("compat", "fixed"):
        raise ValueError("radius mode must be 'compat' or 'fixed'")
    _radius_mode = mode


def _build_sphere_neighbor_impl(database: torch.Tensor, query: torch.Tensor, radius: float,
                           nn_sample: int) -> Tuple[torch.Tensor, torch.Tensor, torch.Tensor]:
    _lib.require_device(database, query)
    if database.dim() != 3 or database.shape[2] != 3:
        raise ValueError("Shape of database points requires to be (batch, npoint, 3)")
    if query.dim() != 3 or query.shape[2] != 3:
        raise ValueError("Shape of query points requires to be (batch, mpoint, 3)")
    database, query = _lib.f32(database), _lib.f32(query)
    B, N, _ = database.shape
    M = query.shape[1]
    nn_index = _lib.empty((B, M, nn_sample), torch.int32, database.device)
    nn_count = _lib.empty((B, M), torch.int32, database.device)
    nn_dist = _lib.empty((B, M, nn_sample), torch.float32, database.device)
    l = _lib.lib()
    sws, swsb = _search_workspace(l, B, N, M, database.device)
    fn = l.sph3d_build_sphere_neighbor_fixed_ws if _radius_mode == "fixed" else l.sph3d_build_sphere_neighbor_ws
    _lib.check(fn(
        B, N, M, nn_sample, radius, _lib.ptr(database), _lib.ptr(query),
        _lib.ptr(nn_index), _lib.ptr(nn_count), _lib.ptr(nn_dist), _lib.ptr(sws), swsb, _lib.stream_ptr()))
    return nn_index, nn_count, nn_dist


def _search_workspace(l, B, N, M, device):
    nbytes = l.sph3d_build_sphere_neighbor_workspace(B, N, M)
    if not nbytes:
        return None, 0
    return _lib.scratch(nbytes, device, slot=1), nbytes


_build_sphere_neighbor = torch.library.custom_op("sph3d::build_sphere_neighbor", mutates_args=())(_build_sphere_neighbor_impl)


@_build_sphere_neighbor.register_fake
def _(database, query, radius, nn_sample):
    B, M = query.shape[0], query.shape[1]
    return (database.new_empty((B, M, nn_sample), dtype=torch.int32),
            database.new_empty((B, M), dtype=torch.int32),
            database.new_empty((B, M, nn_sample), dtype=torch.float32))


def _build_cube_neighbor_impl(database: torch.Tensor, query: torch.Tensor, length: float, nn_sample: int,
                         grid_size: int) -> Tuple[torch.Tensor, torch.Tensor]:
    _lib.require_device(database, query)
    if database.dim() != 3 or database.shape[2] != 3:
        raise ValueError("Shape of database points requires to be (batch, npoint, 3)")
    if query.dim() != 3 or query.shape[2] != 3:
        raise ValueError("Shape of query points requires to be (batch, mpoint, 3)")
    database, query = _lib.f32(database), _lib.f32(query)
    B, N, _ = database.shape
    M = query.shape[1]
    nn_index = torch.empty((B, M, nn_sample, 2), dtype=torch.int32, device=database.device)
    nn_count = torch.empty((B, M), dtype=torch.int32, device=database.device)
    _lib.check(_lib.lib().sph3d_build_cube_neighbor(
        B, N, M, grid_size, nn_sample, length, _lib.ptr(database), _lib.ptr(query),
        _lib.ptr(nn_index), _lib.ptr(nn_count), _lib.stream_ptr()))
    return nn_index, nn_count


_build_cube_neighbor = torch.library.custom_op("sph3d::build_cube_neighbor", mutates_args=())(_build_cube_neighbor_impl)


@_build_cube_neighbor.register_fake
def _(database, query, length, nn_sample, grid_size):
    B, M = query.shape[0], query.shape[1]
    return (database.new_empty((B, M, nn_sample, 2), dtype=torch.int32),
            database.new_empty((B, M), dtype=torch.int32))


def build_sphere_neighbor(database, query, radius=0.1, dilation_rate=None, nnsample=100):
    database = database[:, :, 0:3]
    query = query[:, :, 0:3]
    if dilation_rate is not None:
        radius = dilation_rate * radius
    return _build_sphere_neighbor_impl(database, query, float(radius), int(nnsample))


def build_cube_neighbor(database, query, length=0.1, dilation_rate=None, nnsample=100, gridsize=3):
    database = database[:, :, 0:3]
    query = query[:, :, 0:3]
    if dilation_rate is not None:
        length = dilation_rate * length
    return _build_cube_neighbor_impl(database, query, float(length), int(nnsample), int(gridsize))


def build_sphere_graph(xyz, radius, nnsample, kernel, with_transpose=True):
    from . import _tgraph
    xyz = _lib.f32(xyz[:, :, 0:3])
    _lib.require_device(xyz)
    if _radius_mode == "fixed":
        raise ValueError("build_sphere_graph implements the reference (compat) radius semantics only")
    n, p, q = (int(v) for v in kernel)
    B, N, _ = xyz.shape
    K = int(nnsample)
    F = n * p * q + 1
    dev = xyz.device
    nn_index = _lib.empty((B, N, K), torch.int32, dev)
    nn_count = _lib.empty((B, N), torch.int32, dev)
    nn_dist = _lib.empty((B, N, K), torch.float32, dev)
    filt = _lib.empty((B, N, K), torch.int32, dev)
    l = _lib.lib()
    ws, wsb = None, 0
    if with_transpose:
        wsb = l.sph3d_graph_transpose_workspace(B, N, N, K, F)
        ws = torch.empty((max(wsb, 1),), dtype=torch.uint8, device=dev)
    from . import tf_buildkernel
    sws, swsb = _search_workspace(l, B, N, N, dev)
    _lib.check(l.sph3d_build_sphere_graph_ws(
        B, N, N, K, float(radius), n, p, q, 1 if tf_buildkernel._atan2 == "ocml" else 0, _lib.ptr(xyz), _lib.ptr(xyz),
        _lib.ptr(nn_index), _lib.ptr(nn_count), _lib.ptr(nn_dist), _lib.ptr(filt), _lib.ptr(ws), wsb, _lib.ptr(sws), swsb,
        _lib.stream_ptr()))
    if with_transpose:
        _tgraph.transpose(nn_index, nn_count, N, bin_index=filt, num_bins=F, counted_workspace=ws)
    return nn_index, nn_count, nn_dist, filt


def build_sphere_neighbor_counted(database, query, radius, nnsample):
    from . import _tgraph
    database = _lib.f32(database[:, :, 0:3])
    query = _lib.f32(query[:, :, 0:3])
    _lib.require_device(database, query)
    if _radius_mode == "fixed":
        raise ValueError("build_sphere_neighbor_counted implements the reference (compat) radius semantics only")
    B, N, _ = database.shape
    M = query.shape[1]
    K = int(nnsample)
    dev = database.device
    nn_index = _lib.empty((B, M, K), torch.int32, dev)
    nn_count = _lib.empty((B, M), torch.int32, dev)
    nn_dist = _lib.empty((B, M, K), torch.float32, dev)
    l = _lib.lib()
    wsb = l.sph3d_graph_transpose_workspace(B, N, M, K, 1)
    ws = torch.empty((max(wsb, 1),), dtype=torch.uint8, device=dev)
    sws, swsb = _search_workspace(l, B, N, M, dev)
    _lib.check(l.sph3d_build_sphere_graph_ws(B, N, M, K, float(radius), 0, 0, 0, 0, _lib.ptr(database), _lib.ptr(query),
                                             _lib.ptr(nn_index), _lib.ptr(nn_count), _lib.ptr(nn_dist), _lib.ptr(None), _lib.ptr(ws),
                                             wsb, _lib.ptr(sws), swsb, _lib.stream_ptr()))
    _tgraph.transpose(nn_index, nn_count, N, counted_workspace=ws)
    return nn_index, nn_count, nn_dist
```

Before: 2092.

## Add LDS-resident small-shape neighbor search kernel and skip unused distance outputs

Adds an nnsmall kernel for small point sets (N up to 4096). It stages the database coordinates in LDS as SoA and does a brute-force ballot-based radius search with four queries per wave, which replaces the grid or reference path for the coarse layers. Neighbor emission is factored into a shared helper that skips computing and writing distances when the caller passes a null nn_dist. The S3DIS harness now requests graphs without distances wherever they are unused. Risks are LDS pressure and occupancy for larger N, and making sure the skipped distance outputs are truly never consumed.

```diff
diff --git a/include/sph3d.h b/include/sph3d.h
--- a/include/sph3d.h
+++ b/include/sph3d.h
@@ -25,6 +25,7 @@
 
 #define SPH3D_MAX_GROWTH_PASSES 4096
 long long sph3d_nngrid_launches(void);
+long long sph3d_nnsmall_launches(void);
 int sph3d_build_sphere_neighbor(int B, int N, int M, int nn_sample, float radius,
                                 const float* database, const float* query,
                                 int* nn_index, int* nn_count, float* nn_dist,
diff --git a/sph3d_gcn_amd/_lib.py b/sph3d_gcn_amd/_lib.py
--- a/sph3d_gcn_amd/_lib.py
+++ b/sph3d_gcn_amd/_lib.py
@@ -67,6 +67,7 @@
     "sph3d_pointwise_gemm_bnstats_blocks": (_I, [_I] * 3),
     "sph3d_pointwise_gemm_bnstats": (_I, [_I] * 3 + [_P] * 6),
     "sph3d_nngrid_launches": (ctypes.c_longlong, []),
+    "sph3d_nnsmall_launches": (ctypes.c_longlong, []),
     "sph3d_masked_softmax_xent_parts": (_I, [_I]),
     "sph3d_masked_softmax_xent": (_I, [_I, _I, _I] + [_P] * 5 + [_P]),
     "sph3d_adam_step": (_I, [ctypes.c_longlong] + [_P] * 4 + [_F] * 4 + [_I, _P]),
diff --git a/sph3d_gcn_amd/csrc/nngrid.hip b/sph3d_gcn_amd/csrc/nngrid.hip
--- a/sph3d_gcn_amd/csrc/nngrid.hip
+++ b/sph3d_gcn_amd/csrc/nngrid.hip
@@ -12,6 +12,7 @@
 constexpr int kGridMinCells = 512;
 constexpr int kGridMaxK = 256;
 constexpr int kGridMaxPos = 8;
+constexpr int kSmallMaxN = 4096;
 constexpr int kGridReach = 3;
 
 struct GridHdr {
@@ -203,7 +204,7 @@
     return incl - v;
 }
 
-template <bool FUSE>
+template <bool FUSE, bool DIST>
 __global__ __launch_bounds__(64) void nngrid_search_kernel(
     int B, int N, int M, int K, int W, int parts, int fixed, GraphFuse fx, int* __restrict__ flag,
     const GridRadii* __restrict__ radii, const GridHdr* __restrict__ hdr, const int* __restrict__ cellStart,
@@ -305,35 +306,16 @@
             nnCount[row] = cnt;
             if (found == 0) *flag = 1;
         }
-        for (int slot = l16; slot < K; slot += 16) {
-            int id = 0, bin = 0;
-            float dist = 0.0f;
-            if (slot < cnt) {
-                id = list[slot];
-                const float dx = db[(size_t)id * 3] - qx;
-                const float dy = db[(size_t)id * 3 + 1] - qy;
-                const float dz = db[(size_t)id * 3 + 2] - qz;
-                const float d2 = (dx * dx + dy * dy) + dz * dz;
-                dist = sqrtf(sqrtf(d2));
-                if (FUSE) {
-                    if (fx.filt != nullptr)
-                        bin = fx.ocml ? sphere_bin<true>(dx, dy, dz, dist, fx.radius, fx.n, fx.p, fx.q)
-                                      : sphere_bin<false>(dx, dy, dz, dist, fx.radius, fx.n, fx.p, fx.q);
-                    if (fx.deg != nullptr) {
-                        fx.slotPos[row * K + slot] = atomicAdd(&fx.deg[((size_t)b * N + id) * fx.F + bin], 1);
-                        fx.binUsed[bin] = 1;
-                    }
-                }
-            }
-            nnIndex[row * K + slot] = id;
-            nnDist[row * K + slot] = dist;
-            if (FUSE && fx.filt != nullptr) fx.filt[row * K + slot] = bin;
-        }
+        emit_row<FUSE>(l16, 16, K, cnt, row, b, N, qx, qy, qz, DIST, fx, [&](int slot) { return (int)list[slot]; },
+                       [&](int id, float& x, float& y, float& z) {
+                           x = db[(size_t)id * 3]; y = db[(size_t)id * 3 + 1]; z = db[(size_t)id * 3 + 2];
+                       },
+                       nnIndex, nnDist);
     }
 }
 
 constexpr int kDenseQ = 4;
-template <bool FUSE>
+template <bool FUSE, bool DIST>
 __global__ __launch_bounds__(256) void nndense_kernel(
     int B, int N, int M, int K, int j0, int parts, GraphFuse fx, int* __restrict__ flag, const GridRadii* __restrict__ radii,
     const GridHdr* __restrict__ hdr, const float* __restrict__ database, const float* __restrict__ query,
@@ -425,39 +407,157 @@
             nnCount[row] = cnt;
             if (s[c] == 0) *flag = 1;
         }
-        for (int slot = lane; slot < K; slot += 64) {
-            int id = 0, bin = 0;
-            float dist = 0.0f;
-            if (slot < cnt) {
-                id = h[c * K + slot];
-                const float dx = db[(size_t)id * 3] - qx[c];
-                const float dy = db[(size_t)id * 3 + 1] - qy[c];
-                const float dz = db[(size_t)id * 3 + 2] - qz[c];
+        emit_row<FUSE>(lane, 64, K, cnt, row, b, N, qx[c], qy[c], qz[c], DIST, fx, [&](int slot) { return h[c * K + slot]; },
+                       [&](int id, float& x, float& y, float& z) {
+                           x = db[(size_t)id * 3]; y = db[(size_t)id * 3 + 1]; z = db[(size_t)id * 3 + 2];
+                       },
+                       nnIndex, nnDist);
+    }
+}
+
+constexpr int kSmallQ = 4;
+template <bool FUSE, bool DIST>
+__global__ __launch_bounds__(256) void nnsmall_kernel(
+    int B, int N, int M, int K, int parts, float radius, GraphFuse fx, const float* __restrict__ database,
+    const float* __restrict__ query, int* __restrict__ nnIndex, int* __restrict__ nnCount, float* __restrict__ nnDist)
+{
+    extern __shared__ __attribute__((aligned(16))) unsigned char smem[];
+    const int Np = (N + 63) & ~63;
+    float* X = reinterpret_cast<float*>(smem);
+    const float* Y = X + Np;
+    const float* Z = Y + Np;
+    unsigned short* lists = reinterpret_cast<unsigned short*>(X + 3 * (size_t)Np);
+    int* found = reinterpret_cast<int*>(lists + 4 * kSmallQ * (size_t)K);
+    int b, part;
+    xcd_decode((int)blockIdx.x, B, parts, b, part);
+    if (b < 0) return;
+    const int tid = (int)threadIdx.x, lane = lane_id(), w = uniform(tid >> 6);
+    const float* db = database + (size_t)b * N * 3;
+    for (int p = tid; p < N; p += 256) {
+        X[p] = db[(size_t)p * 3];
+        X[Np + p] = db[(size_t)p * 3 + 1];
+        X[2 * Np + p] = db[(size_t)p * 3 + 2];
+    }
+    const float T0 = range_threshold(radius);
+    __syncthreads();
+    const int jw = (part * 4 + w) * kSmallQ;
+    if (jw >= M) return;
+    unsigned short* h = lists + (size_t)w * kSmallQ * K;
+    float qx[kSmallQ], qy[kSmallQ], qz[kSmallQ];
+    int s[kSmallQ];
+#pragma unroll
+    for (int c = 0; c < kSmallQ; c++) {
+        const bool live = jw + c < M;
+        const size_t row = (size_t)b * M + (live ? jw + c : jw);
+        qx[c] = query[row * 3]; qy[c] = query[row * 3 + 1]; qz[c] = query[row * 3 + 2];
+        s[c] = live ? 0 : K;
+    }
+    for (int base = 0; base < N; base += 64) {
+        bool open = false;
+#pragma unroll
+        for (int c = 0; c < kSmallQ; c++) open = open || s[c] < K;
+        if (!open) break;
+        const int i = base + lane;
+        const float x = X[i], y = Y[i], z = Z[i];
+#pragma unroll
+        for (int c = 0; c < kSmallQ; c++) {
+            if (s[c] < K) {
+                const float dx = x - qx[c], dy = y - qy[c], dz = z - qz[c];
                 const float d2 = (dx * dx + dy * dy) + dz * dz;
-                dist = sqrtf(sqrtf(d2));
-                if (FUSE) {
-                    if (fx.filt != nullptr)
-                        bin = fx.ocml ? sphere_bin<true>(dx, dy, dz, dist, fx.radius, fx.n, fx.p, fx.q)
-                                      : sphere_bin<false>(dx, dy, dz, dist, fx.radius, fx.n, fx.p, fx.q);
-                    if (fx.deg != nullptr) {
-                        fx.slotPos[row * K + slot] = atomicAdd(&fx.deg[((size_t)b * N + id) * fx.F + bin], 1);
-                        fx.binUsed[bin] = 1;
-                    }
+                const bool hit = i < N && d2 < T0;
+                const unsigned long long m = __builtin_amdgcn_ballot_w64(hit);
+                if (m != 0ull) {
+                    const int pos = s[c] + prefix_popc(m);
+                    if (hit && pos < K) h[c * K + pos] = (unsigned short)i;
+                    s[c] += __popcll(m);
                 }
             }
-            nnIndex[row * K + slot] = id;
-            nnDist[row * K + slot] = dist;
-            if (FUSE && fx.filt != nullptr) fx.filt[row * K + slot] = bin;
-        }
+        }
+    }
+#pragma unroll
+    for (int c = 0; c < kSmallQ; c++) {
+        if (s[c] != 0) continue;
+        float r = radius;
+        for (int pass = 1; pass < SPH3D_MAX_GROWTH_PASSES && s[c] == 0; pass++) {
+            r = (float)((double)r + 0.05);
+            const float T = range_threshold(r);
+            for (int base = 0; base < N && s[c] < K; base += 64) {
+                const int i = base + lane;
+                const float dx = X[i] - qx[c], dy = Y[i] - qy[c], dz = Z[i] - qz[c];
+                const float d2 = (dx * dx + dy * dy) + dz * dz;
+                const bool hit = i < N && d2 < T;
+                const unsigned long long m = __builtin_amdgcn_ballot_w64(hit);
+                if (m != 0ull) {
+                    const int pos = s[c] + prefix_popc(m);
+                    if (hit && pos < K) h[c * K + pos] = (unsigned short)i;
+                    s[c] += __popcll(m);
+                }
+            }
+        }
+    }
+    if (lane == 0) {
+#pragma unroll
+        for (int c = 0; c < kSmallQ; c++) found[w * kSmallQ + c] = s[c];
+    }
+    __builtin_amdgcn_fence(__ATOMIC_RELEASE, "wavefront");
+    __builtin_amdgcn_wave_barrier();
+#pragma unroll 1
+    for (int c = 0; c < kSmallQ && jw + c < M; c++) {
+        const size_t row = (size_t)b * M + jw + c;
+        const int sc = found[w * kSmallQ + c];
+        const int cnt = sc < K ? sc : K;
+        if (lane == 0) nnCount[row] = cnt;
+        const float cx = query[row * 3], cy = query[row * 3 + 1], cz = query[row * 3 + 2];
+        emit_row<FUSE>(lane, 64, K, cnt, row, b, N, cx, cy, cz, DIST, fx, [&](int slot) { return (int)h[c * K + slot]; },
+                       [&](int id, float& px, float& py, float& pz) { px = X[id]; py = Y[id]; pz = Z[id]; },
+                       nnIndex, nnDist);
     }
 }
 
 static std::atomic<long long> g_grid_launches{0};
+static std::atomic<long long> g_small_launches{0};
+
+static bool grid_shape(int N, int M)
+{
+    return !(N < 1024 || N > 65536 || M < 64 || M > kMaxPositions * kRefBlock || (long long)N * M < (1LL << 22));
+}
+static bool small_shape(int B, int N, int M, int K, int fixed)
+{
+    return !fixed && B <= kRefGrid && M <= kRefBlock && N <= kSmallMaxN && K <= kGridMaxK &&
+           (N < 1024 || (long long)N * M < (1LL << 22));
+}
+
+bool nnsmall_takes(int B, int N, int M, int K, int fixed) { return small_shape(B, N, M, K, fixed); }
+
+int nnsmall_search(int B, int N, int M, int K, float radius, int fixed, const float* database, const float* query, int* nn_index,
+                   int* nn_count, float* nn_dist, const GraphFuse* fuse, hipStream_t st)
+{
+    if (!small_shape(B, N, M, K, fixed)) return 0;
+    const int parts = (M + 4 * kSmallQ - 1) / (4 * kSmallQ);
+    const int Np = (N + 63) & ~63;
+    const size_t listBytes = (size_t)4 * kSmallQ * K * 2;
+    const size_t lds = (size_t)3 * Np * 4 + listBytes + 4 * kSmallQ * 4;
+    GraphFuse fx{};
+    if (fuse != nullptr) fx = *fuse;
+    int rc = SPH3D_OK;
+#define SPH3D_SMALL(FU, DI)                                                                                                   \
+    rc = launch_lds(nnsmall_kernel<FU, DI>, dim3(xcd_grid(B, parts)), dim3(256), lds, st, "nnsmall", B, N, M, K, parts, radius, fx, \
+                    database, query, nn_index, nn_count, nn_dist)
+    const bool dist = nn_dist != nullptr;
+    if (fuse != nullptr) { if (dist) SPH3D_SMALL(true, true); else SPH3D_SMALL(true, false); }
+    else { if (dist) SPH3D_SMALL(false, true); else SPH3D_SMALL(false, false); }
+#undef SPH3D_SMALL
+    if (rc) return rc;
+    rc = check_launch("nnsmall_search");
+    if (rc) return rc;
+    g_small_launches.fetch_add(1, std::memory_order_relaxed);
+    return 1;
+}
 
 size_t nngrid_workspace_bytes(int B, int N, int M)
 {
     if (B <= 0 || N <= 0 || M <= 0) return 0;
-    if (N < 1024 || N > 65536 || M < 64 || M > kMaxPositions * kRefBlock || (long long)N * M < (1LL << 22)) return 0;
+    if (!grid_shape(N, M)) return 0;
     const size_t hdrBytes = 1024 + sizeof(GridHdr) * (size_t)B;
     const size_t csBytes = sizeof(int) * (size_t)B * (kGridMaxCells + 1);
     const size_t ptBytes = sizeof(float4) * (size_t)B * N;
@@ -470,7 +570,7 @@
                   int* nn_count, float* nn_dist, const GraphFuse* fuse, hipStream_t st, const int** gate, int* grid_done,
                   void* workspace, size_t workspace_bytes, bool library_scratch)
 {
-    if (N < 1024 || N > 65536 || M < 64 || M > kMaxPositions * kRefBlock || (long long)N * M < (1LL << 22) || K > kGridMaxK ||
+    if (!grid_shape(N, M) || K > kGridMaxK ||
         (!fixed && B > kRefGrid && ((M >= kRefBlock && M % kRefBlock != 0) ||
                                     ((B + kRefGrid - 1) / kRefGrid) * ((M + kRefBlock - 1) / kRefBlock) > kMaxPositions)))
         return 0;
@@ -520,13 +620,15 @@
     const size_t lds = (size_t)4 * W * 4 + 4 * 64 * 8 + (size_t)4 * K * 2;
     GraphFuse fx{};
     if (fuse != nullptr) fx = *fuse;
-#define SPH3D_GRID(FU)                                                                                                      \
+#define SPH3D_GRID(FU, DI)                                                                                                  \
     do {                                                                                                                    \
-        auto kern = nngrid_search_kernel<FU>;                                                                               \
+        auto kern = nngrid_search_kernel<FU, DI>;                                                                           \
         hipLaunchKernelGGL(kern, dim3(xcd_grid(B, parts)), dim3(64), lds, st, B, N, M, K, W, parts, fixed, fx, flag, radii, \
                            hdr, cellStart, pts, qorder, database, query, nn_index, nn_count, nn_dist);                      \
     } while (0)
-    if (fuse != nullptr) SPH3D_GRID(true); else SPH3D_GRID(false);
+    const bool dist = nn_dist != nullptr;
+    if (fuse != nullptr) { if (dist) SPH3D_GRID(true, true); else SPH3D_GRID(true, false); }
+    else { if (dist) SPH3D_GRID(false, true); else SPH3D_GRID(false, false); }
 #undef SPH3D_GRID
     int j0 = M;
     if (!fixed) {
@@ -538,12 +640,12 @@
     if (j0 < M) {
         const int dparts = (M - j0 + 4 * kDenseQ - 1) / (4 * kDenseQ);
         const size_t dlds = sizeof(int) * 4 * kDenseQ * (size_t)K;
-        if (fuse != nullptr)
-            hipLaunchKernelGGL(nndense_kernel<true>, dim3(xcd_grid(B, dparts)), dim3(256), dlds, st, B, N, M, K, j0, dparts, fx, flag,
-                               radii, hdr, database, query, nn_index, nn_count, nn_dist);
-        else
-            hipLaunchKernelGGL(nndense_kernel<false>, dim3(xcd_grid(B, dparts)), dim3(256), dlds, st, B, N, M, K, j0, dparts, fx, flag,
-                               radii, hdr, database, query, nn_index, nn_count, nn_dist);
+#define SPH3D_DENSE(FU, DI)                                                                                                 \
+    hipLaunchKernelGGL((nndense_kernel<FU, DI>), dim3(xcd_grid(B, dparts)), dim3(256), dlds, st, B, N, M, K, j0, dparts, fx, flag, \
+                       radii, hdr, database, query, nn_index, nn_count, nn_dist)
+        if (fuse != nullptr) { if (dist) SPH3D_DENSE(true, true); else SPH3D_DENSE(true, false); }
+        else { if (dist) SPH3D_DENSE(false, true); else SPH3D_DENSE(false, false); }
+#undef SPH3D_DENSE
     }
     rc = check_launch("nngrid_search");
     if (rc) return rc;
@@ -556,3 +658,4 @@
 }
 
 extern "C" long long sph3d_nngrid_launches(void) { return sph3d::g_grid_launches.load(std::memory_order_relaxed); }
+extern "C" long long sph3d_nnsmall_launches(void) { return sph3d::g_small_launches.load(std::memory_order_relaxed); }
diff --git a/sph3d_gcn_amd/csrc/nnquery.hip b/sph3d_gcn_amd/csrc/nnquery.hip
--- a/sph3d_gcn_amd/csrc/nnquery.hip
+++ b/sph3d_gcn_amd/csrc/nnquery.hip
@@ -42,6 +42,7 @@
 {
     const int kstart = (gate != nullptr && *gate == 0) ? gridDone : 0;
     if ((long long)kstart * kRefBlock >= M) return;
+    const bool wantDist = nnDist != nullptr;
     extern __shared__ __attribute__((aligned(16))) float lds[];
     int* lhits = reinterpret_cast<int*>(lds + 3 * ((chunkN + 127) & ~127));
     float* lthr = reinterpret_cast<float*>(lhits + (DEFER ? kWavesPerWG * CPW * K : 0));
@@ -235,11 +236,11 @@
                                     const size_t o = ((size_t)i * M + j[c]) * K;
                                     if (hit0 && pos0 < K) {
                                         nnIndex[o + pos0] = c0 + base + lane;
-                                        nnDist[o + pos0] = sqrtf(sqrtf(d2.x));
+                                        if (wantDist) nnDist[o + pos0] = sqrtf(sqrtf(d2.x));
                                     }
                                     if (hit1 && pos1 < K) {
                                         nnIndex[o + pos1] = c0 + base + 64 + lane;
-                                        nnDist[o + pos1] = sqrtf(sqrtf(d2.y));
+                                        if (wantDist) nnDist[o + pos1] = sqrtf(sqrtf(d2.y));
                                     }
                                     s[c] += __popcll(m0) + __popcll(m1);
                                     act[c] = s[c] < K;
@@ -262,34 +263,16 @@
                         if (lane == 0) nnCount[row] = cnt;
                         if (DEFER) {
                             const int* h = lhits + (wave * CPW + c) * K;
-                            for (int slot = lane; slot < K; slot += 64) {
-                                int id = 0, bin = 0;
-                                float dist = 0.0f;
-                                if (slot < cnt) {
-                                    id = h[slot];
-                                    const float dx = dbi[(size_t)id * 3] - qx[c];
-                                    const float dy = dbi[(size_t)id * 3 + 1] - qy[c];
-                                    const float dz = dbi[(size_t)id * 3 + 2] - qz[c];
-                                    const float d2 = (dx * dx + dy * dy) + dz * dz;
-                                    dist = sqrtf(sqrtf(d2));
-                                    if (FUSE) {
-                                        if (fx.filt != nullptr)
-                                            bin = fx.ocml ? sphere_bin<true>(dx, dy, dz, dist, fx.radius, fx.n, fx.p, fx.q)
-                                                          : sphere_bin<false>(dx, dy, dz, dist, fx.radius, fx.n, fx.p, fx.q);
-                                        if (fx.deg != nullptr) {
-                                            fx.slotPos[row * K + slot] = atomicAdd(&fx.deg[((size_t)i * N + id) * fx.F + bin], 1);
-                                            fx.binUsed[bin] = 1;
-                                        }
-                                    }
-                                }
-                                nnIndex[row * K + slot] = id;
-                                nnDist[row * K + slot] = dist;
-                                if (FUSE && fx.filt != nullptr) fx.filt[row * K + slot] = bin;
-                            }
+                            emit_row<FUSE>(lane, 64, K, cnt, row, i, N, qx[c], qy[c], qz[c], wantDist, fx,
+                                           [&](int slot) { return h[slot]; },
+                                           [&](int id, float& x, float& y, float& z) {
+                                               x = dbi[(size_t)id * 3]; y = dbi[(size_t)id * 3 + 1]; z = dbi[(size_t)id * 3 + 2];
+                                           },
+                                           nnIndex, nnDist);
                         } else {
                             for (int slot = cnt + lane; slot < K; slot += 64) {
                                 nnIndex[row * K + slot] = 0;
-                                nnDist[row * K + slot] = 0.0f;
+                                if (wantDist) nnDist[row * K + slot] = 0.0f;
                             }
                         }
                         j[c] += kRefBlock;
@@ -394,6 +377,26 @@
 
 using namespace sph3d;
 
+struct ChainPlan { int cpw; size_t hb; int chunkN; bool multi; };
+static ChainPlan chain_plan(int B, int N, int M, int nn_sample)
+{
+    ChainPlan pl;
+    const long long chains = (long long)(B < kRefGrid ? B : kRefGrid) * (M < kRefBlock ? M : kRefBlock);
+    pl.cpw = chains >= 256LL * kWavesPerWG * 4 ? 4 : (chains >= 256LL * kWavesPerWG * 2 ? 2 : 1);
+    pl.hb = hits_bytes(pl.cpw, nn_sample);
+    int maxChunk = (int)((160 * 1024 - kThrTable * 4 - pl.hb) / 12) & ~127;
+    if (maxChunk > kMaxChunk) maxChunk = kMaxChunk;
+    pl.chunkN = N < maxChunk ? N : maxChunk;
+    pl.multi = N > pl.chunkN;
+    if (pl.multi) {
+        pl.hb = hits_bytes(1, nn_sample);
+        maxChunk = (int)((160 * 1024 - kThrTable * 4 - pl.hb) / 12) & ~127;
+        if (maxChunk > kMaxChunk) maxChunk = kMaxChunk;
+        pl.chunkN = maxChunk;
+    }
+    return pl;
+}
+
 static int sphere_neighbor(int fixed, int B, int N, int M, int nn_sample, float radius,
                            const float* database, const float* query,
                            int* nn_index, int* nn_count, float* nn_dist,
@@ -406,19 +409,15 @@
     SPH3D_REQUIRE(B >= 0 && N > 0 && M >= 0, "BuildSphereNeighbor: bad dims B=%d N=%d M=%d", B, N, M);
     if (B == 0 || M == 0) return SPH3D_OK;
     hipStream_t st = as_stream(stream);
-    const long long chains = (long long)(B < kRefGrid ? B : kRefGrid) * (M < kRefBlock ? M : kRefBlock);
-    const int cpw = chains >= 256LL * kWavesPerWG * 4 ? 4 : (chains >= 256LL * kWavesPerWG * 2 ? 2 : 1);
-    size_t hb = hits_bytes(cpw, nn_sample);
-    int maxChunk = (int)((160 * 1024 - kThrTable * 4 - hb) / 12) & ~127;
-    if (maxChunk > kMaxChunk) maxChunk = kMaxChunk;
-    int chunkN = N < maxChunk ? N : maxChunk;
-    const bool multi = N > chunkN;
-    if (multi) {
-        hb = hits_bytes(1, nn_sample);
-        maxChunk = (int)((160 * 1024 - kThrTable * 4 - hb) / 12) & ~127;
-        if (maxChunk > kMaxChunk) maxChunk = kMaxChunk;
-        chunkN = maxChunk;
-    }
+    const int sm = nnsmall_search(B, N, M, nn_sample, radius, fixed, database, query, nn_index, nn_count, nn_dist, fuse, st);
+    if (sm != 0) {
+        if (fused) *fused = fuse != nullptr;
+        return sm < 0 ? sm : SPH3D_OK;
+    }
+    const ChainPlan pl = chain_plan(B, N, M, nn_sample);
+    const int cpw = pl.cpw, chunkN = pl.chunkN;
+    const size_t hb = pl.hb;
+    const bool multi = pl.multi;
     if (fused) *fused = (fuse != nullptr) && hb != 0;
     if (hb == 0) fuse = nullptr;
     const int* gate = nullptr;
@@ -498,6 +497,9 @@
     } else {
         SPH3D_REQUIRE(transpose_workspace != nullptr, "build_sphere_graph: without bins the call must count (workspace)");
     }
+    SPH3D_REQUIRE(!binned || nn_dist != nullptr || nn_sample <= 0 || B <= 0 || N <= 0 || M <= 0 ||
+                      nnsmall_takes(B, N, M, nn_sample, 0) || chain_plan(B, N, M, nn_sample).hb != 0,
+                  "build_sphere_graph: nn_sample=%d is binned by a kernel of its own, which reads nn_dist", nn_sample);
     const int F = binned ? n * p * q + 1 : 1;
     GraphFuse fx{};
     fx.n = n; fx.p = p; fx.q = q; fx.F = F;
diff --git a/sph3d_gcn_amd/csrc/nnquery.hpp b/sph3d_gcn_amd/csrc/nnquery.hpp
--- a/sph3d_gcn_amd/csrc/nnquery.hpp
+++ b/sph3d_gcn_amd/csrc/nnquery.hpp
@@ -1,5 +1,6 @@
 #pragma once
 #include "common.hpp"
+#include "sphere_bin.hpp"
 
 namespace sph3d {
 
@@ -48,6 +49,45 @@
     int ocml;
 };
 
+template <bool FUSE, class IdOf, class PointOf>
+__device__ __forceinline__ void emit_row(int l, int lanes, int K, int cnt, size_t row, int b, int N, float qx, float qy, float qz,
+                                         bool wantDist, const GraphFuse& fx, IdOf idOf, PointOf pointOf,
+                                         int* __restrict__ nnIndex, float* __restrict__ nnDist)
+{
+    const bool wantBin = FUSE && fx.filt != nullptr;
+    const bool wantGeom = wantDist || wantBin;
+    for (int slot = l; slot < K; slot += lanes) {
+        int id = 0, bin = 0;
+        float dist = 0.0f;
+        if (slot < cnt) {
+            id = idOf(slot);
+            if (wantGeom) {
+                float px, py, pz;
+                pointOf(id, px, py, pz);
+                const float dx = px - qx;
+                const float dy = py - qy;
+                const float dz = pz - qz;
+                const float d2 = (dx * dx + dy * dy) + dz * dz;
+                dist = sqrtf(sqrtf(d2));
+                if (wantBin)
+                    bin = fx.ocml ? sphere_bin<true>(dx, dy, dz, dist, fx.radius, fx.n, fx.p, fx.q)
+                                  : sphere_bin<false>(dx, dy, dz, dist, fx.radius, fx.n, fx.p, fx.q);
+            }
+            if (FUSE && fx.deg != nullptr) {
+                fx.slotPos[row * K + slot] = atomicAdd(&fx.deg[((size_t)b * N + id) * fx.F + bin], 1);
+                fx.binUsed[bin] = 1;
+            }
+        }
+        nnIndex[row * K + slot] = id;
+        if (wantDist) nnDist[row * K + slot] = dist;
+        if (wantBin) fx.filt[row * K + slot] = bin;
+    }
+}
+
+int nnsmall_search(int B, int N, int M, int K, float radius, int fixed, const float* database, const float* query, int* nn_index,
+                   int* nn_count, float* nn_dist, const GraphFuse* fuse, hipStream_t stream);
+bool nnsmall_takes(int B, int N, int M, int K, int fixed);
+
 int nngrid_search(int B, int N, int M, int K, float radius, int fixed, const float* database, const float* query, int* nn_index,
                   int* nn_count, float* nn_dist, const GraphFuse* fuse, hipStream_t stream, const int** gate, int* grid_done,
                   void* workspace, size_t workspace_bytes, bool library_scratch);
diff --git a/sph3d_gcn_amd/harness/s3dis_net.py b/sph3d_gcn_amd/harness/s3dis_net.py
--- a/sph3d_gcn_amd/harness/s3dis_net.py
+++ b/sph3d_gcn_amd/harness/s3dis_net.py
@@ -190,7 +190,10 @@
         return dict(intra_idx=idx, intra_cnt=cnt, filt_idx=filt)
 
     def _bw_kw(self):
-        return {} if self.need_backward else {"with_transpose": False}
+        kw = {} if self.need_backward else {"with_transpose": False}
+        if self.xyz_layers[0].is_cuda:
+            kw["with_dist"] = False
+        return kw
 
     def _make_pool(self, l, g):
         fused = getattr(s3g_util, "gather_pooling_graph", None)
@@ -211,9 +214,12 @@
         xyz_c, xyz_unpool = self.xyz_layers[L - l], self.xyz_layers[L - 1 - l]
         intra_idx, intra_cnt, intra_dst, filt_idx = s3g_util.build_intra_graph(xyz_c, radius, uplimit, c.kernel, **self._bw_kw())
         from .. import tf_nnquery
-        if (self.need_backward and xyz_c.is_cuda and c.unpool_method == 'mean' and s3g_util.neighbor_fn is s3g_util.build_sphere_neighbor
-                and tf_nnquery.get_radius_mode() == "compat"):
-            inter_idx, inter_cnt, inter_dst = tf_nnquery.build_sphere_neighbor_counted(xyz_c, xyz_unpool, radius, uplimit)
+        ours = xyz_c.is_cuda and c.unpool_method == 'mean' and s3g_util.neighbor_fn is s3g_util.build_sphere_neighbor
+        if self.need_backward and ours and tf_nnquery.get_radius_mode() == "compat":
+            inter_idx, inter_cnt, inter_dst = tf_nnquery.build_sphere_neighbor_counted(xyz_c, xyz_unpool, radius, uplimit,
+                                                                                       with_dist=False)
+        elif ours:
+            inter_idx, inter_cnt, inter_dst = tf_nnquery.build_sphere_neighbor_nodist(xyz_c, xyz_unpool, radius, uplimit)
         else:
             inter_idx, inter_cnt, inter_dst = s3g_util.neighbor_fn(xyz_c, xyz_unpool, radius=radius, nnsample=uplimit)
         return dict(intra_idx=intra_idx, intra_cnt=intra_cnt, filt_idx=filt_idx, inter_idx=inter_idx,
diff --git a/sph3d_gcn_amd/sph3gcn_util.py b/sph3d_gcn_amd/sph3gcn_util.py
--- a/sph3d_gcn_amd/sph3gcn_util.py
+++ b/sph3d_gcn_amd/sph3gcn_util.py
@@ -180,10 +180,10 @@
     return intra_idx, intra_cnt, intra_dst, inter_idx, inter_cnt, inter_dst
 
 
-def build_intra_graph(xyz, radius, nn_uplimit, kernel, with_transpose=True):
+def build_intra_graph(xyz, radius, nn_uplimit, kernel, with_transpose=True, with_dist=True):
     from . import tf_nnquery
     if xyz.is_cuda and neighbor_fn is build_sphere_neighbor and tf_nnquery.get_radius_mode() == "compat":
-        return tf_nnquery.build_sphere_graph(xyz, radius, nn_uplimit, kernel, with_transpose=with_transpose)
+        return tf_nnquery.build_sphere_graph(xyz, radius, nn_uplimit, kernel, with_transpose=with_transpose, with_dist=with_dist)
     idx, cnt, dst = neighbor_fn(xyz, xyz, radius=radius, nnsample=nn_uplimit)
     return idx, cnt, dst, spherical_kernel(xyz, xyz, idx, cnt, dst, radius, kernel=kernel)
 
diff --git a/sph3d_gcn_amd/tf_nnquery.py b/sph3d_gcn_amd/tf_nnquery.py
--- a/sph3d_gcn_amd/tf_nnquery.py
+++ b/sph3d_gcn_amd/tf_nnquery.py
@@ -20,6 +20,10 @@
 
 def _build_sphere_neighbor_impl(database: torch.Tensor, query: torch.Tensor, radius: float,
                            nn_sample: int) -> Tuple[torch.Tensor, torch.Tensor, torch.Tensor]:
+    return _sphere_neighbor(database, query, radius, nn_sample, True)
+
+
+def _sphere_neighbor(database, query, radius, nn_sample, with_dist):
     _lib.require_device(database, query)
     if database.dim() != 3 or database.shape[2] != 3:
         raise ValueError("Shape of database points requires to be (batch, npoint, 3)")
@@ -30,7 +34,7 @@
     M = query.shape[1]
     nn_index = _lib.empty((B, M, nn_sample), torch.int32, database.device)
     nn_count = _lib.empty((B, M), torch.int32, database.device)
-    nn_dist = _lib.empty((B, M, nn_sample), torch.float32, database.device)
+    nn_dist = _lib.empty((B, M, nn_sample), torch.float32, database.device) if with_dist else None
     l = _lib.lib()
     sws, swsb = _search_workspace(l, B, N, M, database.device)
     fn = l.sph3d_build_sphere_neighbor_fixed_ws if _radius_mode == "fixed" else l.sph3d_build_sphere_neighbor_ws
@@ -102,7 +106,11 @@
     return _build_cube_neighbor_impl(database, query, float(length), int(nnsample), int(gridsize))
 
 
-def build_sphere_graph(xyz, radius, nnsample, kernel, with_transpose=True):
+def build_sphere_neighbor_nodist(database, query, radius, nnsample):
+    return _sphere_neighbor(database[:, :, 0:3], query[:, :, 0:3], float(radius), int(nnsample), False)
+
+
+def build_sphere_graph(xyz, radius, nnsample, kernel, with_transpose=True, with_dist=True):
     from . import _tgraph
     xyz = _lib.f32(xyz[:, :, 0:3])
     _lib.require_device(xyz)
@@ -115,7 +123,7 @@
     dev = xyz.device
     nn_index = _lib.empty((B, N, K), torch.int32, dev)
     nn_count = _lib.empty((B, N), torch.int32, dev)
-    nn_dist = _lib.empty((B, N, K), torch.float32, dev)
+    nn_dist = _lib.empty((B, N, K), torch.float32, dev) if with_dist else None
     filt = _lib.empty((B, N, K), torch.int32, dev)
     l = _lib.lib()
     ws, wsb = None, 0
@@ -133,7 +141,7 @@
     return nn_index, nn_count, nn_dist, filt
 
 
-def build_sphere_neighbor_counted(database, query, radius, nnsample):
+def build_sphere_neighbor_counted(database, query, radius, nnsample, with_dist=True):
     from . import _tgraph
     database = _lib.f32(database[:, :, 0:3])
     query = _lib.f32(query[:, :, 0:3])
@@ -146,7 +154,7 @@
     dev = database.device
     nn_index = _lib.empty((B, M, K), torch.int32, dev)
     nn_count = _lib.empty((B, M), torch.int32, dev)
-    nn_dist = _lib.empty((B, M, K), torch.float32, dev)
+    nn_dist = _lib.empty((B, M, K), torch.float32, dev) if with_dist else None
     l = _lib.lib()
     wsb = l.sph3d_graph_transpose_workspace(B, N, M, K, 1)
     ws = torch.empty((max(wsb, 1),), dtype=torch.uint8, device=dev)
```

After: 2123, median of 5. 1.01x the previous value.
